# microsoft/GenerativeImage2Text

Hardware: AMD Instinct MI355X
Metric: captions/sec whole-node (GIT_BASE 224px bs=64/GPU greedy len=20) (higher is better)
Workload: dtype f16; 1 GPU; GIT_BASE 224px bs=64/GPU greedy max_len=20 frames=1; global_batch=64, parallelism=dp1, decode_steps_per_caption=19, seq_len_returned=20, hip_graph=True, contexts_in_flight=4, layernorm_folded=True, library=libgitmi_f16.so, encoder_chains=2, schedule=mixed

## Files before the change

### generativeimage2text_amd/csrc/abi_ops.hip

```cpp
#include "../../include/gitmi.h"
#include "abi_common.h"
#include "gitmi_common.h"
#include "launchers.h"

#include <hip/hip_runtime.h>

using namespace gitmi;

#ifdef GITMI_EXPERIMENT
#include "../../include/gitmi_experiment.h"
#define GITMI_EXP_EXPORT extern "C"
#else
#define GITMI_EXP_EXPORT [[maybe_unused]] static
#endif

static inline int round_up(int x, int m) { return (x + m - 1) / m * m; }

extern "C" int gitmi_operand_dtype(void);
static const char* dtype_name(int dtype) {
    return dtype == GITMI_DTYPE_F32 ? "fp32" : dtype == GITMI_DTYPE_BF16 ? "bf16" : dtype == GITMI_DTYPE_F16 ? "fp16" : "unknown";
}
static int check_dtype(const char* op, const char* arg, int dtype) {
    if (dtype == GITMI_DTYPE_F32 || dtype == gitmi_operand_dtype()) return 0;
    return fail("%s: %s is %s (%d), but this library's 16-bit operands are %s (libgitmi%s.so)", op, arg, dtype_name(dtype), dtype,
                dtype_name(gitmi_operand_dtype()), gitmi_operand_dtype() == GITMI_DTYPE_F16 ? "_f16" : "");
}

extern "C" int gitmi_op_gemm(const void* A, const void* W, const float* bias, const float* residual, void* C, int M,
                             int N, int K, int lda, int ldc, int in_dtype, int out_dtype, int act, void* stream) {
    GemmArgs g{};
    g.A = A; g.W = W; g.bias = bias; g.res = residual; g.C = C;
    g.M = M; g.N = N; g.K = K; g.lda = lda; g.ldc = ldc; g.ldr = ldc; g.act = act;
    RCK(check_dtype("op_gemm", "in_dtype", in_dtype));
    const bool in_f32 = in_dtype == GITMI_DTYPE_F32;
    if ((in_f32 && K % 16) || (!in_f32 && K % 64)) return fail("op_gemm: K must be a multiple of %d", in_f32 ? 16 : 64);
    if (out_dtype == GITMI_DTYPE_F16_STREAM) {
        if (in_f32) return fail("op_gemm: fp16 stream rows need 16-bit operands");
        g.out_f16 = 1;
    } else {
        RCK(check_dtype("op_gemm", "out_dtype", out_dtype));
    }
    HIPCK(launch_gemm(g, in_f32, out_dtype == GITMI_DTYPE_F32, (hipStream_t)stream));
    return 0;
}
extern "C" int gitmi_op_gemm_ln(const void* A, const void* W, const float* bias, const float* colsum, const float* ln_part,
                                float ln_eps, const void* residual, const float* res_part, const float* res_gamma,
                                const float* res_beta, float res_eps, void* C, float* part_out, int M, int N, int K, int act,
                                void* stream) {
    GemmArgs g{};
    g.A = A; g.W = W; g.bias = bias; g.C = C;
    g.M = M; g.N = N; g.K = K; g.lda = K; g.ldc = N; g.ldr = N; g.act = act;
    if (K % 64) return fail("op_gemm_ln: K must be a multiple of 64");
    if (ln_part) {
        if (!colsum || residual || part_out || res_part) return fail("op_gemm_ln: consumer form takes colsum and no residual / partial output");
        g.ln_part = (const float2*)ln_part; g.ln_nparts = (K + 255) / 256; g.ln_colsum = colsum; g.ln_inv_d = 1.0f / (float)K; g.ln_eps = ln_eps;
    } else {
        if (!part_out && !res_part) return fail("op_gemm_ln: neither a consumer (ln_part) nor a producer (part_out / res_part)");
        g.out_f16 = 1;
        g.res = (const float*)residual;
        g.part_out = (float2*)part_out;
        if (res_part) {
            g.res_part = (const float2*)res_part; g.res_nparts = (N + 255) / 256; g.res_gamma = res_gamma; g.res_beta = res_beta;
            g.res_inv_d = 1.0f / (float)N; g.res_eps = res_eps;
        }
    }
    if (!gemm_uses_p8(g, false, false))
        return fail("op_gemm_ln: the folded forms exist in gemm_p8_kernel only (more than 512 rows, N %% 256 == 0, K >= 128)");
    if (launch_gemm(g, false, false, (hipStream_t)stream) != hipSuccess)
        return fail("op_gemm_ln: launch refused (the folded forms are built into the fp16-operand library only)");
    return 0;
}
extern "C" int gitmi_op_layernorm(const float* x, const float* gamma, const float* beta, float eps, void* y_t,
                                  float* y_f32, int rows, int D, int out_dtype, void* stream) {
    if (y_t) RCK(check_dtype("op_layernorm", "out_dtype", out_dtype));
    HIPCK(launch_layernorm(x, D, gamma, beta, eps, nullptr, y_t, D, out_dtype == GITMI_DTYPE_F32, y_f32, D, rows, D, 0, 0,
                           0, (hipStream_t)stream));
    return 0;
}
extern "C" int gitmi_op_attention(const void* qkv, void* out, int B, int N, int H, int dtype, int impl, void* stream) {
    RCK(check_dtype("op_attention", "dtype", dtype));
    const size_t esz = dtype == GITMI_DTYPE_F32 ? 4 : 2;
    const int D = H * 64;
    AttnFullArgs a{};
    a.q = qkv;
    a.k = (const char*)qkv + (size_t)D * esz;
    a.v = (const char*)qkv + (size_t)2 * D * esz;
    a.out = out;
    a.ldq = a.ldk = a.ldv = 3 * D;
    a.ldo = D;
    a.N = N; a.H = H; a.scale = 0.125f;
    HIPCK(launch_attn_full(a, B, dtype == GITMI_DTYPE_F32, impl, (hipStream_t)stream));
    return 0;
}

#ifdef GITMI_EXPERIMENT
static int g_dgemm_dbg = 0;
GITMI_EXP_EXPORT int gitmi_debug_set_dgemm(int dbg) { g_dgemm_dbg = dbg; return 0; }
#else
static const int g_dgemm_dbg = 0;
#endif
extern "C" int gitmi_op_dgemm(const void* A, const void* W, const float* bias, const float* colsum, const float* stats,
                              int strips, float eps, void* C, int c_frag, int M, int N, int K, int act, int strips_per_wg,
                              void* stream) {
    if (c_frag && N % 32) return fail("op_dgemm: a fragment-major output needs N %% 32 == 0");
    const DLn ln{(const float2*)stats, strips, 1.0f / (float)K, eps, nullptr, nullptr};
    DGemmArgs g = dgemm_ln(A, W, bias, colsum, stats ? &ln : nullptr, C, c_frag, act, M, N, K);
    g.dbg = g_dgemm_dbg;
    g.strips_per_wg = strips_per_wg;
    if (K % 32) return fail("op_dgemm: K must be a multiple of 32");
    HIPCK(launch_dgemm(g, (hipStream_t)stream));
    return 0;
}
extern "C" int gitmi_op_dgemm_res(const void* A, const void* W, const float* bias, const float* res_x, const float* res_stats,
                                  int res_strips, const float* res_gamma, const float* res_beta, float res_eps,
                                  float* x_out, void* xb_out, float* stats_out, int M, int N, int K, void* stream) {
    const DLn res_ln{(const float2*)res_stats, res_strips, 1.0f / (float)N, res_eps, res_gamma, res_beta};
    DGemmArgs g = dgemm_to_stream(A, W, bias, res_x, res_stats ? &res_ln : nullptr, x_out, xb_out, (float2*)stats_out, M, N, K);
    g.dbg = g_dgemm_dbg;
    if (K % 32 || N % 16) return fail("op_dgemm_res: need K %% 32 == 0 and N %% 16 == 0");
    HIPCK(launch_dgemm(g, (hipStream_t)stream));
    return 0;
}
GITMI_EXP_EXPORT int gitmi_debug_dgemm_form(const void* A, int a_rows, const void* W, const float* bias, const float* colsum,
                                            const float* stats, int strips, float eps, void* C, int c_frag, int act,
                                            const float* res_x, const float* res_stats, int res_strips, const float* res_gamma,
                                            const float* res_beta, float res_eps, float* x_out, void* xb_out, float* stats_out,
                                            int M, int N, int K, int rows_per_wg, int strips_per_wg, int no_row_walk,
                                            void* stream) {
    if (!A || !W || !bias) return fail("debug_dgemm_form: null argument (A, W, bias)");
    if (M < 0 || N < 0 || K < 0) return fail("debug_dgemm_form: M=%d N=%d K=%d", M, N, K);
    if ((C != nullptr) == (x_out != nullptr)) return fail("debug_dgemm_form: exactly one of C and x_out selects the epilogue");
    if (K % 32) return fail("debug_dgemm_form: K must be a multiple of 32 (K=%d)", K);
    if (a_rows < round_up(M, 64)) return fail("debug_dgemm_form: a_rows=%d, but M=%d rows are loaded as %d", a_rows, M, round_up(M, 64));
    if (rows_per_wg < 0 || strips_per_wg < 0) return fail("debug_dgemm_form: rows_per_wg=%d strips_per_wg=%d", rows_per_wg, strips_per_wg);
    DGemmArgs g;
    if (C) {
        if (res_x || res_stats || xb_out || stats_out) return fail("debug_dgemm_form: residual arguments with the C epilogue");
        if (c_frag && N % 32) return fail("debug_dgemm_form: c_frag needs N %% 32 == 0 (N=%d)", N);
        if (stats) {
            if (!colsum) return fail("debug_dgemm_form: stats without colsum");
            if (strips < 1 || strips > 64) return fail("debug_dgemm_form: strips=%d outside [1, 64]", strips);
        }
        const DLn ln{(const float2*)stats, strips, 1.0f / (float)K, eps, nullptr, nullptr};
        g = dgemm_ln(A, W, bias, colsum, stats ? &ln : nullptr, C, c_frag, act, M, N, K);
    } else {
        if (stats || colsum || c_frag || act) return fail("debug_dgemm_form: consumer arguments with the x_out epilogue");
        if (N % 16) return fail("debug_dgemm_form: the x_out epilogue needs N %% 16 == 0 (N=%d)", N);
        if (!xb_out || !stats_out || !res_x) return fail("debug_dgemm_form: the x_out epilogue needs xb_out, stats_out and res_x");
        if (res_stats) {
            if (!res_gamma || !res_beta) return fail("debug_dgemm_form: res_stats without res_gamma / res_beta");
            if (res_strips < 1 || res_strips > 64) return fail("debug_dgemm_form: res_strips=%d outside [1, 64]", res_strips);
        }
        const DLn res_ln{(const float2*)res_stats, res_strips, 1.0f / (float)N, res_eps, res_gamma, res_beta};
        g = dgemm_to_stream(A, W, bias, res_x, res_stats ? &res_ln : nullptr, x_out, xb_out, (float2*)stats_out, M, N, K);
    }
    g.rows_per_wg = rows_per_wg; g.strips_per_wg = strips_per_wg; g.no_row_walk = no_row_walk;
    HIPCK(launch_dgemm(g, (hipStream_t)stream));
    return 0;
}
static VocabArgs vocab_op_args(const void* A, const void* W, const float* bias, const float* colsum, const float* stats, int strips,
                               float eps, int M, int V, int K, int cols_per_wg, float* part_val, int* part_idx, float* part_lse,
                               float* logits_out, int max_wgs) {
    VocabArgs v{};
    v.max_wgs = max_wgs;
    v.A = (const unsigned short*)A; v.lda = K; v.W = (const unsigned short*)W; v.bias = bias;
// ... 95 lines not shown
        HIPCK(hipMemcpy(node.data(), child_node, node.size() * sizeof(int), hipMemcpyDeviceToHost));
        for (int i = 0; i < n_edges; ++i)
            if (node[i] < 0 || node[i] >= n_nodes) return fail("debug_trie_select: edge %d leads to node %d of %d", i, node[i], n_nodes);
    }
    HIPCK(hipMemcpy(cur.data(), cursor, cur.size() * sizeof(int), hipMemcpyDeviceToHost));
    for (int b = 0; b < B; ++b)
        if (cur[b] < -1 || cur[b] >= n_nodes) return fail("debug_trie_select: cursor %d of sentence %d outside [-1, %d)", cur[b], b, n_nodes);
    const TrieArgs tr{child_off, child_tok, child_node, cursor};
    HIPCK(launch_trie_select(logits, ldl, V, ids, ld_ids, cur_len, plen, eos, tr, B, part_val, part_idx, (float2*)part_lse, s));
    return 0;
}
GITMI_EXP_EXPORT int gitmi_debug_sample_rows(const float* logits, int R, int V, float temperature, int top_k, float top_p, int ndraw,
                                             uint64_t seed, int step, float* draw_logprob, int* draw_token, float* filtered_out,
                                             int ldl, const int* ids, int ld_ids, int cur_len, float rep_penalty, int stride,
                                             void* stream) {
    if (!logits || !draw_logprob || !draw_token) return fail("debug_sample_rows: null argument");
    if (R < 1 || V < 1 || ldl < V) return fail("debug_sample_rows: R=%d V=%d ldl=%d", R, V, ldl);
    RCK(check_history("debug_sample_rows", ids, ld_ids, cur_len));
    float2* lse = nullptr;
    HIPCK(hipMalloc((void**)&lse, (size_t)R * sizeof(float2)));
    hipError_t err = launch_sample_rows(logits, ldl, V, R, temperature, top_k, top_p, ndraw, seed, step, draw_logprob, draw_token, lse,
                                        filtered_out, ids, ld_ids, cur_len, rep_penalty, stride, (hipStream_t)stream);
    if (err == hipSuccess) err = hipStreamSynchronize((hipStream_t)stream);
    hipFree(lse);
    HIPCK(err);
    return 0;
}

GITMI_EXP_EXPORT int gitmi_debug_set_gemm_impl(int impl) {
    if (!set_gemm_impl(impl)) return fail("debug_set_gemm_impl: unknown selector %d (low byte: -1, 0 or 9)", impl);
    return 0;
}

GITMI_EXP_EXPORT int gitmi_debug_gemm_form(const void* A, int lda, const void* W, const float* bias, const void* res, int ldr, void* C,
                                           int ldc, int M, int N, int K, int act, int in_dtype, int out_dtype, int shared,
                                           const float* ln_part, const float* colsum, float ln_eps, float* part_out,
                                           const float* res_part, const float* res_gamma, const float* res_beta, float res_eps,
                                           void* stream) {
    if (!A || !W || !C) return fail("debug_gemm_form: null argument (A, W, C)");
    if (M < 0 || N < 1 || K < 1) return fail("debug_gemm_form: M=%d N=%d K=%d", M, N, K);
    if (lda < K) return fail("debug_gemm_form: lda=%d < K=%d", lda, K);
    if (ldc < N) return fail("debug_gemm_form: ldc=%d < N=%d", ldc, N);
    if (res && ldr < N) return fail("debug_gemm_form: ldr=%d < N=%d", ldr, N);
    if (act < GITMI_ACT_NONE || act > GITMI_ACT_GELU_ERF) return fail("debug_gemm_form: act=%d", act);
    RCK(check_dtype("debug_gemm_form", "in_dtype", in_dtype));
    const bool in_f32 = in_dtype == GITMI_DTYPE_F32;
    if ((in_f32 && K % 16) || (!in_f32 && K % 64)) return fail("debug_gemm_form: K must be a multiple of %d (K=%d)", in_f32 ? 16 : 64, K);
    GemmArgs g{};
    g.A = A; g.W = W; g.bias = bias; g.res = (const float*)res; g.C = C;
    g.M = M; g.N = N; g.K = K; g.lda = lda; g.ldc = ldc; g.ldr = res ? ldr : 0; g.act = act;
    g.shared = shared ? 1 : 0;
    if (out_dtype == GITMI_DTYPE_F16_STREAM) {
        if (in_f32) return fail("debug_gemm_form: fp16 stream rows need 16-bit operands");
        g.out_f16 = 1;
    } else {
        RCK(check_dtype("debug_gemm_form", "out_dtype", out_dtype));
    }
    const bool out_f32 = out_dtype == GITMI_DTYPE_F32;
    const bool consumer = ln_part != nullptr, producer = part_out != nullptr || res_part != nullptr;
    if (colsum && !consumer) return fail("debug_gemm_form: colsum without ln_part");
    if ((res_gamma || res_beta) && !res_part) return fail("debug_gemm_form: res_gamma / res_beta without res_part");
    if (consumer || producer) {
#ifndef GITMI_OPS_F16
        return fail("debug_gemm_form: the folded-LayerNorm forms are built into the fp16-operand library only");
#endif
        if (consumer && producer) return fail("debug_gemm_form: consumer (ln_part) and producer (part_out / res_part) arguments in one launch");
        if (consumer) {
            if (!colsum) return fail("debug_gemm_form: ln_part without colsum");
            if (res || in_f32 || out_f32 || g.out_f16) return fail("debug_gemm_form: the consumer writes operand-type rows and takes no residual");
            if (K > 1024) return fail("debug_gemm_form: row partials cover K <= 1024 (K=%d)", K);
            g.ln_part = (const float2*)ln_part; g.ln_nparts = (K + 255) / 256; g.ln_colsum = colsum; g.ln_inv_d = 1.0f / (float)K; g.ln_eps = ln_eps;
        } else {
            if (!g.out_f16 || act != GITMI_ACT_NONE) return fail("debug_gemm_form: the producer writes fp16 stream rows and has no activation");
            if (N > 1024) return fail("debug_gemm_form: row partials cover N <= 1024 (N=%d)", N);
            g.part_out = (float2*)part_out;
            if (res_part) {
                if (!res || !res_gamma || !res_beta) return fail("debug_gemm_form: res_part without res / res_gamma / res_beta");
                g.res_part = (const float2*)res_part; g.res_nparts = (N + 255) / 256; g.res_gamma = res_gamma; g.res_beta = res_beta;
                g.res_inv_d = 1.0f / (float)N; g.res_eps = res_eps;
            }
        }
        if (!gemm_uses_p8(g, false, false))
            return fail("debug_gemm_form: the folded forms exist in gemm_p8_kernel only (more than 512 rows, N %% 256 == 0, K >= 128, 16-byte aligned rows)");
    }
    HIPCK(launch_gemm(g, in_f32, out_f32, (hipStream_t)stream));
    return 0;
}

extern "C" int gitmi_op_attn_decode(const void* qkv, const void* img_k, const void* img_v, void* txt_k, void* txt_v,
                                    const int* kv_src, void* out, int B, int H, int N_img, int T_max, int pos, int beams,
                                    int dtype, int dbg, void* stream) {
    RCK(check_dtype("op_attn_decode", "dtype", dtype));
    AttnDecodeArgs a{};
    a.qkv = qkv; a.img_k = img_k; a.img_v = img_v; a.txt_k = txt_k; a.txt_v = txt_v; a.out = out;
    a.kv_src = kv_src; a.ld_src = T_max; a.d = H * 64; a.N_img = N_img; a.T_max = T_max; a.pos = pos; a.beams = beams;
    a.scale = 0.125f; a.dbg = dbg & 0xffff; a.waves_per_pair = (dbg >> 16) & 3; a.stream_wgs = dbg >> 18;
    if (dtype == GITMI_DTYPE_F32) {
        HIPCK(launch_attn_decode(a, B, H, (hipStream_t)stream));
        return 0;
    }
    a.N_pad = round_up(N_img, 32);
    HIPCK(launch_attn_decode_mfma(a, B, H, (hipStream_t)stream));
    return 0;
}
extern "C" int gitmi_op_kv_repack(const void* qkv_rows, void* kf, void* vt, int B, int N, int H, void* stream) {
    HIPCK(launch_kv_repack_frag(qkv_rows, kf, vt, B, N, round_up(N, 32), H, H * 64, (hipStream_t)stream));
    return 0;
}

GITMI_EXP_EXPORT int gitmi_debug_attention_ragged(const void* qkv, void* out, const int* ntok, int B, int N, int H, int dtype, int impl,
                                                  void* stream) {
    if (!ntok) return fail("debug_attention_ragged: ntok is required");
    const size_t esz = dtype == GITMI_DTYPE_F32 ? 4 : 2;
    const int D = H * 64;
    AttnFullArgs a{};
    a.q = qkv;
    a.k = (const char*)qkv + (size_t)D * esz;
    a.v = (const char*)qkv + (size_t)2 * D * esz;
    a.out = out;
    a.ldq = a.ldk = a.ldv = 3 * D;
    a.ldo = D;
    a.N = N; a.H = H; a.scale = 0.125f; a.ntok = ntok;
    HIPCK(launch_attn_full(a, B, dtype == GITMI_DTYPE_F32, impl, (hipStream_t)stream));
    return 0;
}
GITMI_EXP_EXPORT int gitmi_debug_attn_decode_form(const void* qkv, const void* img_k, const void* img_v, void* txt_k, void* txt_v,
                                                  const int* kv_src, void* out, const int* ntok, const int* img_of, int n_images,
                                                  int B, int H, int N_img, int T_max, int pos, int beams, int dtype, int out_frag,
                                                  int pairs_per_wg, int waves_per_pair, int stream_wgs, void* stream) {
    RCK(check_dtype("debug_attn_decode_form", "dtype", dtype));
    if (!qkv || !img_k || !img_v || !txt_k || !txt_v || !kv_src || !out) return fail("debug_attn_decode_form: null argument");
    if (beams < 1 || beams > 8) return fail("debug_attn_decode_form: beams=%d outside [1, 8]", beams);
    if (n_images < 1) return fail("debug_attn_decode_form: n_images=%d", n_images);
    if (B < 1 || H < 1 || N_img < 1 || pos < 0 || pos >= T_max)
        return fail("debug_attn_decode_form: B=%d H=%d N_img=%d pos=%d T_max=%d", B, H, N_img, pos, T_max);
    if (out_frag && dtype == GITMI_DTYPE_F32) return fail("debug_attn_decode_form: out_frag needs 16-bit rows");
    if (ntok && stream_wgs > 0) return fail("debug_attn_decode_form: the streaming kernel does not serve ragged batches (ntok)");
    AttnDecodeArgs a{};
    a.qkv = qkv; a.img_k = img_k; a.img_v = img_v; a.txt_k = txt_k; a.txt_v = txt_v; a.out = out;
    a.kv_src = kv_src; a.ld_src = T_max; a.d = H * 64; a.N_img = N_img; a.T_max = T_max; a.pos = pos; a.beams = beams;
    a.scale = 0.125f; a.ntok = ntok; a.img_of = img_of; a.out_frag = out_frag;
    a.pairs_per_wg = pairs_per_wg; a.waves_per_pair = waves_per_pair; a.stream_wgs = stream_wgs;
    if (dtype == GITMI_DTYPE_F32) {
        HIPCK(launch_attn_decode(a, B, H, (hipStream_t)stream));
        return 0;
    }
    a.N_pad = round_up(N_img, 32);
    HIPCK(launch_attn_decode_mfma(a, B, H, (hipStream_t)stream));
    return 0;
}
GITMI_EXP_EXPORT int gitmi_debug_attn_decode_qkv(const void* x, int x_rows, const void* w, const float* bias, const float* colsum,
                                                 const float* stats, int strips, float eps, const void* img_k, const void* img_v,
                                                 void* txt_k, void* txt_v, const int* kv_src, void* out, const int* ntok,
                                                 const int* img_of, int n_images, int B, int H, int N_img, int T_max, int pos,
                                                 int beams, int dtype, int out_frag, int pairs_per_wg, int waves_per_pair,
                                                 int stream_wgs, void* stream) {
    RCK(check_dtype("debug_attn_decode_qkv", "dtype", dtype));
    if (dtype == GITMI_DTYPE_F32) return fail("debug_attn_decode_qkv: 16-bit operands only (the f32 mode keeps its QKV launch)");
    if (!x || !w || !bias || !img_k || !img_v || !txt_k || !txt_v || !kv_src || !out) return fail("debug_attn_decode_qkv: null argument");
    if (n_images < 1) return fail("debug_attn_decode_qkv: n_images=%d", n_images);
    if (B < 1 || H < 1 || N_img < 1 || pos < 0 || pos >= T_max)
        return fail("debug_attn_decode_qkv: B=%d H=%d N_img=%d pos=%d T_max=%d", B, H, N_img, pos, T_max);
    if (beams != 1) return fail("debug_attn_decode_qkv: beams=%d (beam batches keep the QKV launch)", beams);
    if (ntok) return fail("debug_attn_decode_qkv: ntok (ragged batches keep the QKV launch)");
    if (waves_per_pair == 2) return fail("debug_attn_decode_qkv: waves_per_pair=2 (two-wave pairs keep the QKV launch)");
    if (stream_wgs != 0) return fail("debug_attn_decode_qkv: stream_wgs=%d (the streaming form keeps the QKV launch)", stream_wgs);
// ... 247 lines not shown
```

### generativeimage2text_amd/csrc/engine.hip

```cpp
#include "../../include/gitmi.h"
#include "engine_state.h"

#include <algorithm>
#include <cmath>
#include <cstdarg>
#include <cstdio>
#include <cstring>

using namespace gitmi;

#ifdef GITMI_EXPERIMENT
#include "../../include/gitmi_experiment.h"
#define GITMI_EXP_EXPORT extern "C"
#else
#define GITMI_EXP_EXPORT [[maybe_unused]] static
#endif

static thread_local char g_err[1024] = "";
int gitmi::fail(const char* fmt, ...) {
    va_list ap;
    va_start(ap, fmt);
    vsnprintf(g_err, sizeof(g_err), fmt, ap);
    va_end(ap);
    return 1;
}

static hipEvent_t get_event(gitmi_engine* e) {
    if (e->event_next == e->event_pool.size()) {
        hipEvent_t ev;
        hipEventCreate(&ev);
        e->event_pool.push_back(ev);
    }
    return e->event_pool[e->event_next++];
}
struct SpanGuard {
    gitmi_engine* e; hipStream_t s; size_t idx; bool on;
    SpanGuard(gitmi_engine* e_, hipStream_t s_, int tag, double flops) : e(e_), s(s_), idx(0), on(e_->profiling) {
        if (!on) return;
        TimedSpan sp{get_event(e), get_event(e), tag, flops};
        hipEventRecord(sp.a, s);
        idx = e->spans.size();
        e->spans.push_back(sp);
    }
    ~SpanGuard() { if (on) hipEventRecord(e->spans[idx].b, s); }
};

static bool gemm_tall_tiles(const gitmi_engine* e, int N) {
    if (!e->pol.shared_device) return false;
    return e->pol.gemm_tall == 1 || (e->pol.gemm_tall == 2 && N >= 2048) || (e->pol.gemm_tall == 3 && N < 2048);
}

static double gemm_flops(int M, int N, int K) { return 2.0 * (double)M * (double)N * (double)K; }
static GemmArgs gemm_args(const void* A, int lda, const void* W, const float* bias, const void* res, int ldr, void* C, int ldc,
                          int M, int N, int K, int act) {
    GemmArgs g{};
    g.A = A; g.W = W; g.bias = bias; g.res = (const float*)res; g.C = C;
    g.M = M; g.N = N; g.K = K; g.lda = lda; g.ldc = ldc; g.ldr = ldr; g.act = act;
    return g;
}
static int gemm_run(gitmi_engine* e, hipStream_t s, GemmArgs g, bool in_f32, bool out_f32, int tag) {
    g.shared = gemm_tall_tiles(e, g.N) ? 1 : 0;
    SpanGuard sp(e, s, tag, gemm_flops(g.M, g.N, g.K));
    HIPCK(launch_gemm(g, in_f32, out_f32, s));
    return 0;
}
static int gemm(gitmi_engine* e, hipStream_t s, const void* A, int lda, const void* W, const float* bias,
                const float* res, int ldr, void* C, int ldc, bool out_f32, int M, int N, int K, int act, int tag) {
    return gemm_run(e, s, gemm_args(A, lda, W, bias, res, ldr, C, ldc, M, N, K, act), e->pol.f32, out_f32, tag);
}
static bool on_p8(const void* A, int lda, const void* W, const void* C, int ldc, int M, int N, int K, bool stream_out) {
    GemmArgs g = gemm_args(A, lda, W, nullptr, nullptr, 0, const_cast<void*>(C), ldc, M, N, K, 0);
    g.out_f16 = stream_out ? 1 : 0;
    return gemm_uses_p8(g, false, false);
}
struct Stream {
    void* x = nullptr; int M = 0, D = 0, tag = 0;
    bool fold = false;
    void* t = nullptr;
    float* xn = nullptr;
    float2* parts[2] = {nullptr, nullptr};
    const float2* part = nullptr; const float* gamma = nullptr; const float* beta = nullptr; float eps = 0.f;
};
static float2* stream_part_out(const Stream& st) { return st.part == st.parts[0] ? st.parts[1] : st.parts[0]; }
static void stream_written(Stream& st, const float2* part, const float* gamma, const float* beta, float eps) {
    st.part = part; st.gamma = gamma; st.beta = beta; st.eps = eps;
}
static int ln_gemm(gitmi_engine* e, hipStream_t s, const Stream& st, const Folded& f, const void* W, const float* bias, void* C,
                   int ldc, int col0, int N, int act) {
    const int D = st.D;
    const size_t woff = (size_t)col0 * D * e->pol.esz;
    C = (char*)C + (size_t)col0 * e->pol.esz;
    if (st.fold) {
        GemmArgs g = gemm_args(st.x, D, (const char*)f.w + woff, f.bias + col0, nullptr, 0, C, ldc, st.M, N, D, act);
        g.ln_part = st.part; g.ln_nparts = D / 256; g.ln_colsum = f.colsum + col0; g.ln_inv_d = 1.0f / (float)D; g.ln_eps = st.eps;
        return gemm_run(e, s, g, false, false, st.tag);
    }
    if (e->pol.stream_f16)
        HIPCK(launch_layernorm_s16(st.x, D, st.gamma, st.beta, st.eps, nullptr, st.t, D, false, st.xn, st.xn ? D : 0, st.M, D, 0, 0, 0, s));
    else
        HIPCK(launch_layernorm((const float*)st.x, D, st.gamma, st.beta, st.eps, nullptr, st.t, D, e->pol.f32, st.xn, st.xn ? D : 0, st.M,
                               D, 0, 0, 0, s));
    return gemm(e, s, st.t, D, (const char*)W + woff, bias + col0, nullptr, 0, C, ldc, e->pol.f32, st.M, N, D, act, st.tag);
}
static int gemm_to_stream(gitmi_engine* e, hipStream_t s, Stream& st, const void* A, int lda, const void* W, const float* bias, int K,
                          bool residual, const float* gamma, const float* beta, float eps) {
    const int D = st.D;
    float2* part = gamma ? stream_part_out(st) : nullptr;
    const void* res = !residual ? nullptr : st.xn && !st.fold ? st.xn : st.x;
    GemmArgs g = gemm_args(A, lda, W, bias, res, residual ? D : 0, st.x, D, st.M, D, K, 0);
    g.out_f16 = e->pol.stream_f16 ? 1 : 0;
    if (st.fold) {
        g.part_out = part;
        if (residual && st.xn) {
            g.res_part = st.part; g.res_nparts = D / 256; g.res_gamma = st.gamma; g.res_beta = st.beta;
            g.res_inv_d = 1.0f / (float)D; g.res_eps = st.eps;
        }
    }
    RCK(gemm_run(e, s, g, e->pol.f32, !e->pol.stream_f16, st.tag));
    stream_written(st, part, gamma, beta, eps);
    return 0;
}
static int attn_full_packed(gitmi_engine* e, const void* qkv, void* out, int width, int heads, int N, int batch, const int* ntok,
                            hipStream_t s) {
    AttnFullArgs a{};
    a.q = qkv;
    a.k = (const char*)qkv + (size_t)width * e->pol.esz;
    a.v = (const char*)qkv + (size_t)2 * width * e->pol.esz;
    a.out = out;
    a.ldq = a.ldk = a.ldv = 3 * width;
    a.ldo = width;
    a.N = N; a.H = heads; a.scale = 0.125f;
    a.ntok = ntok;
    HIPCK(launch_attn_full(a, batch, e->pol.f32, e->pol.attn_impl, s));
    return 0;
}
static int dec_layer_tail(gitmi_engine* e, hipStream_t s, const DecLayerW& L, const void* ctx, float* hf, void* ht, float* y, void* u,
                          int M) {
    const int d = e->cfg.dec_hidden, ffn = e->cfg.dec_ffn;
    RCK(gemm(e, s, ctx, d, L.wo, L.bo, hf, d, y, d, true, M, d, d, 0, TAG_GEMM_OTHER));
    HIPCK(launch_layernorm(y, d, L.lnag, L.lnab, 1e-12f, nullptr, ht, d, e->pol.f32, hf, d, M, d, 0, 0, 0, s));
    RCK(gemm(e, s, ht, d, L.w1, L.b1, nullptr, 0, u, ffn, e->pol.f32, M, ffn, d, 2, TAG_GEMM_OTHER));
    RCK(gemm(e, s, u, ffn, L.w2, L.b2, hf, d, y, d, true, M, d, ffn, 0, TAG_GEMM_OTHER));
    HIPCK(launch_layernorm(y, d, L.lnog, L.lnob, 1e-12f, nullptr, ht, d, e->pol.f32, hf, d, M, d, 0, 0, 0, s));
    return 0;
}

extern "C" int gitmi_abi_version(void) { return GITMI_ABI_VERSION; }
extern "C" int gitmi_operand_dtype(void) {
#ifdef GITMI_OPS_F16
    return GITMI_DTYPE_F16;
#else
    return GITMI_DTYPE_BF16;
#endif
}
extern "C" const char* gitmi_last_error(void) { return g_err; }

extern "C" int gitmi_create(const gitmi_config* cfg, int device, gitmi_engine** out) {
    if (!cfg || !out) return fail("gitmi_create: null argument");
    int ndev = 0;
    if (hipGetDeviceCount(&ndev) != hipSuccess || ndev <= 0)
        return fail("gitmi_create: no HIP device available (this engine has no CPU fallback)");
    if (device < 0 || device >= ndev) return fail("gitmi_create: device %d out of range (%d devices)", device, ndev);
    HIPCK(hipSetDevice(device));
    hipDeviceProp_t prop;
    HIPCK(hipGetDeviceProperties(&prop, device));
    if (strncmp(prop.gcnArchName, "gfx950", 6) != 0)
        return fail("gitmi_create: device %d is %s; this library is built for gfx950 (MI355X) only", device,
                    prop.gcnArchName);
    const gitmi_config& c = *cfg;
    if (c.vit_width % c.vit_heads || c.vit_width / c.vit_heads != 64) return fail("ViT head_dim must be 64");
    if (c.dec_hidden % c.dec_heads || c.dec_hidden / c.dec_heads != 64) return fail("decoder head_dim must be 64");
    if (c.image_size % c.patch) return fail("image_size must be a multiple of patch");
    if (c.max_image_pixels < 0 || c.max_image_tokens < 0) return fail("negative image capacity");
    if (c.vit_width > 1024 || c.dec_hidden > 1024) return fail("hidden sizes above 1024 are not supported");
    if (c.vit_width % 64 || c.dec_hidden % 64 || c.dec_ffn % 64) return fail("hidden sizes must be multiples of 64");
    if (c.max_batch < 1 || c.max_beams < 1 || c.max_beams > 8 || c.max_frames < 1 || c.max_text_len < 2)
        return fail("bad capacity (max_batch>=1, 1<=max_beams<=8, max_frames>=1, max_text_len>=2)");
    if (c.max_text_len > c.max_pos) return fail("max_text_len exceeds max_pos");
    if (c.precision != GITMI_PREC_BF16 && c.precision != GITMI_PREC_F32) return fail("bad precision");

    gitmi_engine* e = new gitmi_engine();
    e->cfg = c;
    e->device = device;
    e->pol.f32 = c.precision == GITMI_PREC_F32;
    e->pol.esz = e->pol.f32 ? 4 : 2;
    e->pol.attn_impl = e->pol.f32 ? 0 : 1;
    init_geometry(e);
    e->pol.stream_f16 = !e->pol.f32;
#ifdef GITMI_OPS_F16
    e->pol.ln_fold = !e->pol.f32 && c.vit_width % 256 == 0 && c.dec_hidden % 256 == 0;
#endif
#ifdef GITMI_EXPERIMENT
    if (const char* env = getenv("GITMI_ATTN_IMPL")) e->pol.attn_impl = e->pol.f32 ? 0 : atoi(env);
    if (const char* env = getenv("GITMI_GRAPH")) e->pol.use_graph = atoi(env) != 0;
    if (const char* env = getenv("GITMI_ATTN_DBG")) e->pol.attn_dbg = atoi(env);
    if (const char* env = getenv("GITMI_ATTN_PW")) e->pol.attn_pw = atoi(env);
    if (const char* env = getenv("GITMI_ATTN_NH")) e->pol.attn_nh = atoi(env);
    if (const char* env = getenv("GITMI_ATTN_STREAM")) e->pol.attn_stream = atoi(env);
    if (const char* env = getenv("GITMI_DECODE_SKIP")) e->pol.decode_skip = atoi(env);
    if (const char* env = getenv("GITMI_GEMM_TALL")) e->pol.gemm_tall = atoi(env);
    if (const char* env = getenv("GITMI_DGEMM_ROWS")) e->pol.dgemm_rows = atoi(env);
    if (const char* env = getenv("GITMI_DGEMM_STRIPS")) e->pol.dgemm_strips = atoi(env);
    if (const char* env = getenv("GITMI_DGEMM_NO_ROW_WALK")) e->pol.dgemm_no_row_walk = atoi(env);
    if (const char* env = getenv("GITMI_DGEMM_DBG")) e->pol.dgemm_dbg = atoi(env);
    if (const char* env = getenv("GITMI_VOCAB_WGS")) e->pol.vocab_wgs = atoi(env);
    if (const char* env = getenv("GITMI_SKINNY")) e->pol.skinny = atoi(env) != 0;
    if (const char* env = getenv("GITMI_STREAM_F16")) e->pol.stream_f16 = !e->pol.f32 && atoi(env) != 0;
    if (const char* env = getenv("GITMI_GEMM_IMPL")) set_gemm_impl(atoi(env));
#endif
    e->pol.ln_fold = e->pol.ln_fold && e->pol.stream_f16;
    e->pol.ln_fold_ready = e->pol.ln_fold;
    *out = e;
    return 0;
}

int CapturedGraph::capture(hipStream_t s, const std::function<int()>& fn) {
    reset();
    HIPCK(hipStreamBeginCapture(s, hipStreamCaptureModeThreadLocal));
    const int rc = fn();
    const hipError_t ce = hipStreamEndCapture(s, &graph);
    if (rc != 0 || ce != hipSuccess) reset();
    RCK(rc);
    HIPCK(ce);
    HIPCK(hipGraphInstantiate(&exec, graph, nullptr, nullptr, 0));
    return 0;
}
static void destroy_graph(gitmi_engine* e) {
    for (CapturedGraph* g : {&e->graph_full, &e->graph_decode, &e->graph_follow}) g->reset();
    e->full_slot.valid = e->follow_slot.valid = false;
}
static void drop_resident(gitmi_engine* e) { e->have_feats = e->have_prefill = false; }
static void set_resident(gitmi_engine* e, int B, int F_eff, int stride = 0) {
    e->cur_B = B; e->cur_F = F_eff; e->cur_Nimg = stride > 0 ? stride : F_eff * e->N;
    e->have_feats = true; e->have_prefill = false;
    e->keyed = e->ragged; e->has_context = false;
    e->res_desc.clear();
}
static void set_context(gitmi_engine* e) { e->keyed = e->has_context = true; }
static const int* key_counts(const gitmi_engine* e) { return e->keyed ? e->rg_ntok : nullptr; }
static void set_prefilled(gitmi_engine* e) { e->have_prefill = true; }
static int settle_residency(gitmi_engine* e, const Request& rq, int rc) {
    if (rc != 0 && rq.frames) drop_resident(e);
    return rc;
}

extern "C" void gitmi_destroy(gitmi_engine* e) {
    if (!e) return;
    hipSetDevice(e->device);
    hipDeviceSynchronize();
    if (e->enc_after) {
        auto& w = e->enc_after->enc_watchers;
        w.erase(std::remove(w.begin(), w.end(), e), w.end());
    }
    for (gitmi_engine* w : e->enc_watchers) w->enc_after = nullptr;
    destroy_graph(e);
    if (e->own_stream) hipStreamDestroy(e->own_stream);
    if (e->fence_in) hipEventDestroy(e->fence_in);
    if (e->fence_out) hipEventDestroy(e->fence_out);
    for (auto ev : e->gev)
        if (ev) hipEventDestroy(ev);
    if (e->enc_done) hipEventDestroy(e->enc_done);
    for (auto ev : e->event_pool) hipEventDestroy(ev);
    for (void* p : e->allocs) hipFree(p);
    for (void* p : e->sc_allocs) hipFree(p);
    hipFree(e->at_out); hipFree(e->at_stats); hipFree(e->ctx_tab); hipFree(e->mem_tab); hipFree(e->feat_tab); hipFree(e->ban_words);
    if (e->ban_stage) hipHostFree(e->ban_stage);
    if (e->ban_staged) hipEventDestroy(e->ban_staged);
    if (e->trie_off) hipFree(e->trie_off);
    if (e->trie_tok) hipFree(e->trie_tok);
    if (e->trie_child) hipFree(e->trie_child);
    delete e;
}

extern "C" int gitmi_set_image_shape(gitmi_engine* e, int H, int W, void* stream) {
    if (!e) return fail("null engine");
    if (!e->finalized) return fail("weights not finalized");
    const gitmi_config& c = e->cfg;
    if (H == 0 && W == 0) {
        if (!e->ragged) {
            e->ragged = true;
            e->H = e->W = e->gh = e->gw = 0;
            e->N = e->Nmax;
            drop_resident(e);
        }
        return 0;
    }
    if (H < c.patch || W < c.patch) return fail("image %dx%d is smaller than one %d-pixel patch", H, W, c.patch);
    const int gh = H / c.patch, gw = W / c.patch;
    if ((size_t)H * W > e->max_pixels)
        return fail("image %dx%d exceeds the max_image_pixels capacity (%zu)", H, W, e->max_pixels);
    if (gh * gw + 1 > e->Nmax)
        return fail("a %dx%d token grid exceeds the max_image_tokens capacity (%d)", gh, gw, e->Nmax);
    if (H == e->H && W == e->W && !e->ragged) return 0;
    e->ragged = false;
    HIPCK(hipSetDevice(e->device));
    if (gh == e->g_nat && gw == e->g_nat) {
        e->pos_cur = e->w.pos;
    } else {
        HIPCK(launch_pos_bicubic(e->w.pos, e->pos_var, e->g_nat, gh, gw, c.vit_width, (hipStream_t)stream));
        e->pos_cur = e->pos_var;
    }
    e->H = H; e->W = W; e->gh = gh; e->gw = gw; e->N = gh * gw + 1;
    drop_resident(e);
    return 0;
}

static Stream vit_stream(gitmi_engine* e, int M) {
    const int D = e->cfg.vit_width;
    const VitLayerW& L = e->w.vit[0];
    Stream st;
    st.x = e->v_x; st.M = M; st.D = D; st.tag = TAG_GEMM_VIT; st.t = e->v_h;
    st.fold = e->pol.ln_fold && on_p8(e->v_x, D, L.qkv_f.w, e->v_qkv, 3 * D, M, 3 * D, D, false) &&
              on_p8(e->v_x, D, L.ffn1_f.w, e->v_u, 4 * D, M, 4 * D, D, false) && on_p8(e->v_ctx, D, L.wo, e->v_x, D, M, D, D, true) &&
              on_p8(e->v_u, 4 * D, L.w2, e->v_x, D, M, D, 4 * D, true);
    if (st.fold) st.parts[0] = st.parts[1] = e->v_part;
    return st;
}
static Stream prefill_stream(gitmi_engine* e, int M) {
    const int d = e->cfg.dec_hidden, ffn = e->cfg.dec_ffn, D = e->cfg.vit_width;
    const DecLayerW& L = e->w.dec[0];
    Stream st;
    st.x = e->p_y; st.M = M; st.D = d; st.tag = TAG_GEMM_OTHER; st.t = e->p_ht; st.xn = e->p_hf;
    st.fold = e->pol.ln_fold && on_p8(e->feats, D, e->w.vp_w, e->p_y, d, M, d, D, true) &&
              on_p8(e->p_y, d, L.qkv_pf.w, e->img_kv[0], 3 * d, M, 3 * d, d, false) &&
              on_p8(e->p_y, d, L.qkv_pf.w, e->img_kv[0], 3 * d, M, 2 * d, d, false) &&
              (e->cfg.dec_layers < 2 || (on_p8(e->p_y, d, L.ffn1_pf.w, e->p_u, ffn, M, ffn, d, false) &&
                                         on_p8(e->p_ctx, d, L.wo, e->p_y, d, M, d, d, true) && on_p8(e->p_u, ffn, L.w2, e->p_y, d, M, d, ffn, true)));
    if (st.fold) { st.parts[0] = e->p_part[0]; st.parts[1] = e->p_part[1]; }
    return st;
}

static int encode_frames_impl(gitmi_engine* e, const float* const* frames, int F, int B, float* feats_out,
                              hipStream_t s, int stride = 0) {
    const gitmi_config& c = e->cfg;
    const int D = c.vit_width, N = e->N;
    const int F_eff = c.num_frames > 0 ? std::min(F, c.num_frames) : F;
    const int Nimg = stride > 0 ? stride : F_eff * N;
    drop_resident(e);
    SpanGuard phase(e, s, TAG_VIT, 0);
    const int BI = F_eff * B;
    const int M = BI * N;
    const int g2 = N - 1;
    const size_t slot = (size_t)3 * e->max_pixels;
    if (e->ragged)
        HIPCK(launch_im2col_ragged(e->frame_stage[0], slot, e->rg_meta, e->patches, e->pol.f32, B, N, c.patch, e->Kp, e->Kp_pad, s));
    else
    for (int fr = 0; fr < F_eff; ++fr)
        HIPCK(launch_im2col(frames[fr], (char*)e->patches + (size_t)fr * B * g2 * e->Kp_pad * e->pol.esz, e->pol.f32, B,
                            e->H, e->W, c.patch, e->Kp, e->Kp_pad, s));
    RCK(gemm(e, s, e->patches, e->Kp_pad, e->w.conv_w, nullptr, nullptr, 0, e->patch_out, D, true, BI * g2, D, e->Kp_pad, 0,
             TAG_GEMM_VIT));
    Stream x = vit_stream(e, M);
    float2* part = stream_part_out(x);
    if (e->ragged)
        HIPCK(launch_vit_assemble_ragged(e->patch_out, e->w.cls, e->w.pos, e->g_nat, e->rg_meta, e->w.lnpre_g, e->w.lnpre_b, 1e-5f, e->v_x,
                                         e->pol.stream_f16, BI, N, c.patch, D, part, s));
    else
    HIPCK(launch_vit_assemble_ln(e->patch_out, e->w.cls, e->pos_cur, e->w.lnpre_g, e->w.lnpre_b, 1e-5f, e->v_x, e->pol.stream_f16, BI, N, D,
                                 part, D / 256, s));
    stream_written(x, part, e->w.vit[0].ln1g, e->w.vit[0].ln1b, 1e-5f);
    for (int l = 0; l < c.vit_layers; ++l) {
        const VitLayerW& L = e->w.vit[l];
        const VitLayerW* Ln = l + 1 < c.vit_layers ? &e->w.vit[l + 1] : nullptr;
        RCK(ln_gemm(e, s, x, L.qkv_f, L.wqkv, L.bqkv, e->v_qkv, 3 * D, 0, 3 * D, 0));
        RCK(attn_full_packed(e, e->v_qkv, e->v_ctx, D, c.vit_heads, N, BI, e->ragged ? e->rg_ntok : nullptr, s));
        RCK(gemm_to_stream(e, s, x, e->v_ctx, D, L.wo, L.bo, D, true, L.ln2g, L.ln2b, 1e-5f));
        RCK(ln_gemm(e, s, x, L.ffn1_f, L.w1, L.b1, e->v_u, 4 * D, 0, 4 * D, 1));
        RCK(gemm_to_stream(e, s, x, e->v_u, 4 * D, L.w2, L.b2, 4 * D, true, Ln ? Ln->ln1g : nullptr, Ln ? Ln->ln1b : nullptr, 1e-5f));
    }
    for (int fr = 0; fr < F_eff; ++fr) {
        const float* te = (c.num_frames > 0 && e->pol.use_temb) ? e->w.temb[fr] : nullptr;
        if (e->pol.stream_f16) {
            const char* xs = (const char*)e->v_x + (size_t)fr * B * N * D * 2;
            HIPCK(launch_layernorm_s16(xs, D, e->w.lnpost_g, e->w.lnpost_b, 1e-5f, te, e->feats, D, false, nullptr, 0, B * N, D, N,
                                       Nimg, fr * N, s));
            if (feats_out)
                HIPCK(launch_layernorm_s16(xs, D, e->w.lnpost_g, e->w.lnpost_b, 1e-5f, te, feats_out, D, true, nullptr, 0, B * N, D,
                                           N, Nimg, fr * N, s));
        } else {
            HIPCK(launch_layernorm(e->v_x + (size_t)fr * B * N * D, D, e->w.lnpost_g, e->w.lnpost_b, 1e-5f, te, e->feats, D, e->pol.f32,
                                   feats_out, D, B * N, D, N, Nimg, fr * N, s));
        }
    }
    if (e->ragged) {
        HIPCK(launch_zero_pad_rows(e->feats, e->pol.f32, D, e->rg_ntok, B, N, s));
        if (feats_out) HIPCK(launch_zero_pad_rows(feats_out, true, D, e->rg_ntok, B, N, s));
    }

    set_resident(e, B, F_eff, stride);
    return 0;
}

static int kv_repack(gitmi_engine* e, int l, int B, int Nimg, hipStream_t s) {
    const gitmi_config& c = e->cfg;
    void* kh = e->img_kh[l];
    void* vh = e->img_vh[l];
    if (e->pol.f32) HIPCK(launch_kv_repack(e->img_kv[l], kh, vh, B, Nimg, c.dec_heads, c.dec_hidden, s));
    else HIPCK(launch_kv_repack_frag(e->img_kv[l], kh, vh, B, Nimg, round_up(Nimg, 32), c.dec_heads, c.dec_hidden, s));
    return 0;
}

static int prefill_impl(gitmi_engine* e, hipStream_t s) {
    const gitmi_config& c = e->cfg;
    const int d = c.dec_hidden, ffn = c.dec_ffn, D = c.vit_width;
    const int B = e->cur_B, Nimg = e->cur_Nimg, M = B * Nimg;
    e->have_prefill = false;
    SpanGuard phase(e, s, TAG_PREFILL, 0);
    Stream y = prefill_stream(e, M);
    RCK(gemm_to_stream(e, s, y, e->feats, D, e->w.vp_w, e->w.vp_b, D, false, e->w.vp_lng, e->w.vp_lnb, 1e-5f));
    for (int l = 0; l < c.dec_layers; ++l) {
        const DecLayerW& L = e->w.dec[l];
        const bool last = l + 1 == c.dec_layers;
        const int col0 = last ? d : 0;
        RCK(ln_gemm(e, s, y, L.qkv_pf, L.wqkv, L.bqkv, e->img_kv[l], 3 * d, col0, 3 * d - col0, 0));
        RCK(kv_repack(e, l, B, Nimg, s));
        if (last) break;
        RCK(attn_full_packed(e, e->img_kv[l], e->p_ctx, d, c.dec_heads, Nimg, B, key_counts(e), s));
        RCK(gemm_to_stream(e, s, y, e->p_ctx, d, L.wo, L.bo, d, true, L.lnag, L.lnab, 1e-12f));
        RCK(ln_gemm(e, s, y, L.ffn1_pf, L.w1, L.b1, e->p_u, ffn, 0, ffn, 2));
        RCK(gemm_to_stream(e, s, y, e->p_u, ffn, L.w2, L.b2, ffn, true, L.lnog, L.lnob, 1e-12f));
    }
    set_prefilled(e);
    return 0;
}

#ifdef GITMI_EXPERIMENT
#define GITMI_SKIPPED(e, bit) (((e)->pol.decode_skip & (bit)) != 0)
#else
#define GITMI_SKIPPED(e, bit) false
#endif
static int dgemm(gitmi_engine* e, hipStream_t s, const DGemmArgs& g_in) {
    DGemmArgs g = g_in;
    g.dbg = e->pol.dgemm_dbg;
    g.no_row_walk = e->pol.dgemm_no_row_walk >= 0 ? e->pol.dgemm_no_row_walk : e->pol.shared_device ? 0 : 1;
    g.strips_per_wg = e->pol.dgemm_strips >= 0 ? e->pol.dgemm_strips : e->pol.shared_device ? 2 : 1;
    g.rows_per_wg = e->pol.dgemm_rows > 0 ? e->pol.dgemm_rows : g.M > 64 ? 64 : e->pol.shared_device ? 32 : 16;
    SpanGuard sp(e, s, TAG_GEMM_OTHER, gemm_flops(g.M, g.N, g.K));
    HIPCK(launch_dgemm(g, s));
    return 0;
}

static DGemmArgs dgemm_ln(const void* A, const Folded& f, const DLn* ln, void* C, int c_frag, int act, int M, int N, int K) {
    return dgemm_ln(A, f.w, f.bias, f.colsum, ln, C, c_frag, act, M, N, K);
}

static int decode_layers_impl(gitmi_engine* e, const int* kv_src, int ld_ids, int pos, int R, int beams, hipStream_t s) {
    const gitmi_config& c = e->cfg;
    const int d = c.dec_hidden, ffn = c.dec_ffn;
    const int B = R / beams;
    const bool chain = e->pol.skinny && !e->pol.f32;
    for (int l = 0; l < c.dec_layers; ++l) {
        const DecLayerW& L = e->w.dec[l];
        const DecLayerW* Lp = l > 0 ? &e->w.dec[l - 1] : nullptr;
        const DLn ln_prev{e->stats_o, d / 16, 1.0f / (float)d, 1e-12f, Lp ? Lp->lnog : nullptr, Lp ? Lp->lnob : nullptr};
        const DLn ln_a{e->stats_a, d / 16, 1.0f / (float)d, 1e-12f, L.lnag, L.lnab};
        const DLn* ln_o = Lp ? &ln_prev : nullptr;
        AttnDecodeArgs a{};
        a.qkv = e->d_qkv; a.img_k = e->img_kh[l]; a.img_v = e->img_vh[l]; a.txt_k = e->txt_k[l]; a.txt_v = e->txt_v[l]; a.out = e->d_ctx;
        a.kv_src = kv_src; a.ld_src = ld_ids; a.d = d; a.N_img = e->cur_Nimg; a.T_max = c.max_text_len;
        a.img_of = e->img_identity ? nullptr : e->img_of_dev;
        a.pos = pos; a.beams = beams; a.scale = 0.125f;
        a.out_frag = chain ? 1 : 0;
        a.N_pad = round_up(e->cur_Nimg, 32);
        a.dbg = e->pol.attn_dbg;
        a.waves_per_pair = e->pol.attn_nh;
        a.pairs_per_wg = e->pol.attn_pw > 0 ? e->pol.attn_pw : e->pol.shared_device ? 8 : 4;
        const bool stream_ok = !e->pol.shared_device && a.N_pad <= 8 * 32 && B * c.dec_heads >= 384 && e->pol.attn_nh != 2;
        a.stream_wgs = e->pol.attn_stream >= 0 ? e->pol.attn_stream : stream_ok ? 192 : 0;
        if (e->keyed) { a.ntok = e->rg_ntok; a.stream_wgs = 0; }
        bool qkv_inside = false;
        if (chain) {
            const DGemmArgs g = dgemm_ln(l == 0 ? e->d_ht : e->xo_b, L.qkv_f, ln_o, e->d_qkv, 0, 0, R, 3 * d, d);
            attn_decode_set_qkv(a, g);
            qkv_inside = !GITMI_SKIPPED(e, ~0) && !e->pol.dgemm_dbg && attn_decode_qkv_form(a, B, c.dec_heads) && attn_decode_pairs_per_wg(a, B, c.dec_heads) == 8;
            if (!qkv_inside && !GITMI_SKIPPED(e, 2) && !GITMI_SKIPPED(e, 16)) RCK(dgemm(e, s, g));
        } else {
            RCK(gemm(e, s, e->d_ht, d, L.wqkv, L.bqkv, nullptr, 0, e->d_qkv, 3 * d, e->pol.f32, R, 3 * d, d, 0, TAG_GEMM_OTHER));
        }
        if (e->pol.f32) HIPCK(launch_attn_decode(a, B, c.dec_heads, s));
        else if (qkv_inside) HIPCK(launch_attn_decode_qkv(a, B, c.dec_heads, s));
        else if (!GITMI_SKIPPED(e, 1)) HIPCK(launch_attn_decode_mfma(a, B, c.dec_heads, s));
        if (chain) {
            if (!GITMI_SKIPPED(e, 4))
                RCK(dgemm(e, s, dgemm_to_stream(e->d_ctx, L.wo_p, L.bo, l == 0 ? e->d_hf : e->xo_f, ln_o, e->xa_f, e->xa_b, e->stats_a, R, d, d)));
            if (!GITMI_SKIPPED(e, 2)) RCK(dgemm(e, s, dgemm_ln(e->xa_b, L.ffn1_f, &ln_a, e->d_u, 1, 2, R, ffn, d)));
            if (!GITMI_SKIPPED(e, 4))
                RCK(dgemm(e, s, dgemm_to_stream(e->d_u, L.w2_p, L.b2, e->xa_f, &ln_a, e->xo_f, e->xo_b, e->stats_o, R, d, ffn)));
        } else {
            RCK(dec_layer_tail(e, s, L, e->d_ctx, e->d_hf, e->d_ht, e->d_y, e->d_u, R));
        }
    }
    return 0;
}

static int sample_candidates(gitmi_engine* e, const float* logits, int ldl, int R, int step, hipStream_t s, StepCands* cands,
                             const BanArgs* ban);
static int trie_candidates(gitmi_engine* e, const float* logits, int ldl, int cur_len, hipStream_t s, StepCands* cands);
static float rep_penalty_of(const gitmi_engine* e) {
    const double rp = e->sample.repetition_penalty;
    return (e->ss.kind == GITMI_SEARCH_GENERATOR && rp > 0 && rp != 1.0) ? (float)rp : 0.f;
}
// ... 1321 lines not shown
```

### generativeimage2text_amd/csrc/engine_state.h

```cpp
#pragma once
#include "../../include/gitmi.h"
#include "abi_common.h"
#include "launchers.h"

#include <hip/hip_runtime.h>

#include <functional>
#include <map>
#include <string>
#include <tuple>
#include <vector>

static inline int round_up(int x, int m) { return (x + m - 1) / m * m; }
static inline int keep_best(const gitmi_search& sp) { return sp.num_keep_best > 1 ? sp.num_keep_best : 1; }

struct HostTensor {
    std::vector<float> data;
    std::vector<int64_t> shape;
    float amax = 0.f;
    size_t numel() const { size_t n = 1; for (auto s : shape) n *= (size_t)s; return n; }
};

struct Folded { void* w = nullptr; float* bias = nullptr; float* colsum = nullptr; };

struct VitLayerW {
    void *wqkv = nullptr, *wo = nullptr, *w1 = nullptr, *w2 = nullptr;
    float *bqkv = nullptr, *bo = nullptr, *b1 = nullptr, *b2 = nullptr;
    float *ln1g = nullptr, *ln1b = nullptr, *ln2g = nullptr, *ln2b = nullptr;
    Folded qkv_f;
    Folded ffn1_f;
};
struct DecLayerW {
    void *wqkv = nullptr, *wo = nullptr, *w1 = nullptr, *w2 = nullptr;
    float *bqkv = nullptr, *bo = nullptr, *b1 = nullptr, *b2 = nullptr;
    float *lnag = nullptr, *lnab = nullptr, *lnog = nullptr, *lnob = nullptr;
    Folded qkv_f;
    Folded ffn1_f;
    void *wo_p = nullptr, *w2_p = nullptr;
    Folded qkv_pf, ffn1_pf;
};

struct TimedSpan { hipEvent_t a, b; int tag; double flops; };
enum { TAG_VIT = 0, TAG_PREFILL = 1, TAG_DECODE = 2, TAG_GEMM_VIT = 10, TAG_GEMM_OTHER = 11, TAG_STEP = 20 };

struct GraphKey {
    int B, Q, F, P, kind, k, pn, T, H, W, prefixed, ident, temb, resident, Nimg, keyed; double lp;
    int smp, top_k, nh; double top_p, temp, rp; unsigned long long seed;
    int constrained;
    auto fields() const {
        return std::tie(B, Q, F, P, kind, k, pn, T, H, W, prefixed, ident, temb, resident, Nimg, keyed, lp, smp, top_k, nh, top_p, temp,
                        rp, seed, constrained);
    }
    bool operator==(const GraphKey& o) const { return fields() == o.fields(); }
};
struct GraphSlot { GraphKey key{}; bool valid = false; };

struct CapturedGraph {
    hipGraph_t graph = nullptr;
    hipGraphExec_t exec = nullptr;
    void reset() {
        if (exec) hipGraphExecDestroy(exec);
        if (graph) hipGraphDestroy(graph);
        exec = nullptr, graph = nullptr;
    }
    int capture(hipStream_t s, const std::function<int()>& fn);
    hipError_t launch(hipStream_t s) const { return hipGraphLaunch(exec, s); }
};

struct Request {
    const float* const* frames;
    int F, B, Q, minP, maxP;
    bool prefixed;
    const gitmi_search* sp;
    long long* tokens; float* logprob; int32_t* info;
    int32_t* sent;
};

struct ModelWeights {
    void* conv_w = nullptr;
    float *cls = nullptr, *pos = nullptr, *lnpre_g = nullptr, *lnpre_b = nullptr, *lnpost_g = nullptr, *lnpost_b = nullptr;
    std::vector<VitLayerW> vit;
    std::vector<float*> temb;
    void* vp_w = nullptr;
    float *vp_b = nullptr, *vp_lng = nullptr, *vp_lnb = nullptr;
    float *words_f = nullptr, *positions_f = nullptr, *emb_lng = nullptr, *emb_lnb = nullptr;
    std::vector<DecLayerW> dec;
    void* out_w = nullptr;
    float* out_b = nullptr;
    Folded out_f;
    double dec_weight_bytes = 0;
};

struct Policy {
    bool f32 = false;
    size_t esz = 2;
    int attn_impl = 1;
    bool stream_f16 = false;
    bool ln_fold = false;
    bool ln_fold_ready = false;
    bool skinny = true;
    bool use_graph = true;
    bool use_temb = true;
    bool shared_device = false;
    int attn_dbg = 0, dgemm_dbg = 0;
    int attn_pw = 0;
    int attn_nh = 0;
    int attn_stream = -1;
    int dgemm_no_row_walk = -1;
    int dgemm_strips = -1;
    int vocab_wgs = -1;
    int gemm_tall = 1;
    int dgemm_rows = 0;
    int decode_skip = 0;
};

struct gitmi_engine {
    gitmi_config cfg{};
    ModelWeights w;
    Policy pol;
    int device = 0;
    bool finalized = false;
    gitmi_engine* parent = nullptr;

    std::map<std::string, HostTensor> host_w;
    std::vector<void*> allocs;

    int N = 0, gh = 0, gw = 0, H = 0, W = 0, Kp = 0, Kp_pad = 0;
    int N_nat = 0, g_nat = 0, Nmax = 0;
    size_t max_pixels = 0;
    float* pos_var = nullptr;
    const float* pos_cur = nullptr;
    bool ragged = false;
    int4* rg_meta = nullptr;
    int* rg_ntok = nullptr;
    bool keyed = false;
    bool has_context = false;
    int* ctx_tab = nullptr;
    size_t ctx_tab_ints = 0;
    gitmi::MemoryEntry* mem_tab = nullptr;
    size_t mem_tab_n = 0;
    std::vector<int4> res_desc;
    gitmi::FeaturePiece* feat_tab = nullptr;
    unsigned int* ban_words = nullptr;
    int* ban_stage = nullptr;
    hipEvent_t ban_staged = nullptr;
    int ban_armed = 0;
    bool ban_live = false;

    void *patches = nullptr, *v_h = nullptr, *v_qkv = nullptr, *v_ctx = nullptr, *v_u = nullptr;
    float *patch_out = nullptr, *v_x = nullptr;
    void* feats = nullptr;
    float *p_y = nullptr, *p_hf = nullptr;
    void *p_ht = nullptr, *p_ctx = nullptr, *p_u = nullptr;
    std::vector<void*> img_kv;
    std::vector<void*> img_kh, img_vh;
    float *d_y = nullptr, *d_hf = nullptr, *logits = nullptr;
    void *d_ht = nullptr, *d_qkv = nullptr, *d_ctx = nullptr, *d_u = nullptr;
    std::vector<void*> txt_k, txt_v;
    int ldl = 0;
    float *xa_f = nullptr, *xo_f = nullptr;
    void *xa_b = nullptr, *xo_b = nullptr;
    float2 *stats_a = nullptr, *stats_o = nullptr;
    float* part_val = nullptr; int* part_idx = nullptr; float2* part_lse = nullptr;
    int vocab_cols = 128, vocab_nparts = 1;
    gitmi::SearchState ss{};
    int ss_cur = 0, ss_len = 0;
    long long* start_dev = nullptr;
    int *plen_dev = nullptr, *img_of_dev = nullptr;
    bool img_identity = true;
    int *trie_off = nullptr, *trie_tok = nullptr, *trie_child = nullptr, *trie_cursor = nullptr;
    bool trie_search = false;
    gitmi_search sample{};
    std::vector<int> plen_host, img_of_host;

    int cur_B = 0, cur_F = 0, cur_Nimg = 0;
    bool have_feats = false, have_prefill = false;

    int profile_mode = 0;
    bool profiling = false;
    float2 *v_part = nullptr, *p_part[2] = {nullptr, nullptr};
    hipEvent_t gev[3] = {nullptr, nullptr, nullptr};
    gitmi_engine* enc_after = nullptr;
    std::vector<gitmi_engine*> enc_watchers;
    hipEvent_t enc_done = nullptr;
    double split_encode_ms = 0, split_decode_ms = 0;
    int split_calls = 0, split_steps = 0;
    std::vector<TimedSpan> spans;
    std::vector<hipEvent_t> event_pool;
    size_t event_next = 0;
    double last_decode_step_bytes = 0;

    CapturedGraph graph_full, graph_decode, graph_follow;
    GraphSlot full_slot, follow_slot;
    bool graph_is_split = false;
    std::vector<float*> frame_stage;
    long long* out_tokens = nullptr;
    float* out_lp = nullptr;
    int* out_info = nullptr;
    int* out_sent = nullptr;
    hipStream_t own_stream = nullptr;
    hipEvent_t fence_in = nullptr, fence_out = nullptr;

    size_t sc_rows = 0;
    std::vector<void*> sc_allocs;
    float *sc_hf = nullptr, *sc_y = nullptr, *sc_zt = nullptr;
    void *sc_ht = nullptr, *sc_qkv = nullptr, *sc_ctx = nullptr, *sc_u = nullptr;
    float4* sc_part = nullptr;
    int *sc_tgt = nullptr, *sc_lens = nullptr, *sc_img = nullptr, *sc_bad = nullptr, *sc_info = nullptr;
    float2* sc_out = nullptr;
    size_t tr_out_n = 0;
    int* tr_nodes = nullptr;
    float2* tr_out = nullptr;
    size_t at_floats = 0, at_stat_rows = 0;
    float* at_out = nullptr;
    float2* at_stats = nullptr;
};

namespace gitmi {
void init_geometry(gitmi_engine* e);
}
```

### generativeimage2text_amd/csrc/engine_weights.hip

```cpp
#include "engine_state.h"

#include <algorithm>
#include <cmath>
#include <cstring>

using namespace gitmi;

static int dev_alloc(gitmi_engine* e, void** p, size_t bytes) {
    if (bytes == 0) bytes = 16;
    HIPCK(hipMalloc(p, bytes));
    e->allocs.push_back(*p);
    return 0;
}
template <typename T> static int dev_alloc_t(gitmi_engine* e, T** p, size_t count) {
    return dev_alloc(e, reinterpret_cast<void**>(p), count * sizeof(T));
}

static float half_to_float(uint16_t h) {
    const uint32_t sign = (uint32_t)(h & 0x8000) << 16;
    uint32_t exp = (h >> 10) & 0x1f, man = h & 0x3ff, out;
    if (exp == 0) {
        if (man == 0) out = sign;
        else {
            exp = 127 - 15 + 1;
// ... 41 lines not shown
}

static int get_w(gitmi_engine* e, const std::string& key, std::initializer_list<int64_t> shape, const HostTensor** out) {
    auto it = e->host_w.find(key);
    if (it == e->host_w.end()) return fail("missing weight '%s'", key.c_str());
    size_t want = 1;
    for (auto s : shape) want *= (size_t)s;
    if (it->second.numel() != want) return fail("weight '%s' has %zu elements, expected %zu", key.c_str(), it->second.numel(), want);
    *out = &it->second;
    return 0;
}
static int up_f32(gitmi_engine* e, const std::string& key, std::initializer_list<int64_t> shape, float** dst) {
    const HostTensor* t;
    RCK(get_w(e, key, shape, &t));
    RCK(dev_alloc_t(e, dst, t->numel()));
    HIPCK(hipMemcpy(*dst, t->data.data(), t->numel() * 4, hipMemcpyHostToDevice));
    return 0;
}
static int operand_range_check(gitmi_engine* e, const char* what, float amax) {
#ifdef GITMI_OPS_F16
    if (!e->pol.f32 && amax > 65504.f)
        return fail("'%s': max |w| = %g is outside the fp16 operand range (65504): load this checkpoint with precision "
                    "\"bf16\" or \"f32\"", what, (double)amax);
#endif
    (void)e; (void)what; (void)amax;
    return 0;
}
static int up_mat(gitmi_engine* e, const std::string& key, int64_t rows, int K, int Kpad, void** dst) {
    const HostTensor* t;
    RCK(get_w(e, key, {rows, (int64_t)K}, &t));
    RCK(operand_range_check(e, key.c_str(), t->amax));
    RCK(dev_alloc(e, dst, (size_t)rows * Kpad * e->pol.esz));
    float* tmp = nullptr;
    HIPCK(hipMalloc((void**)&tmp, t->numel() * 4));
    hipError_t err = hipMemcpy(tmp, t->data.data(), t->numel() * 4, hipMemcpyHostToDevice);
    if (err == hipSuccess) err = launch_convert_pad(tmp, *dst, e->pol.f32, (size_t)rows, K, Kpad, 0);
    if (err == hipSuccess) err = hipDeviceSynchronize();
    hipFree(tmp);
    HIPCK(err);
    return 0;
}

void gitmi::init_geometry(gitmi_engine* e) {
    const gitmi_config& c = e->cfg;
    e->g_nat = e->gh = e->gw = c.image_size / c.patch;
    e->N_nat = e->N = e->g_nat * e->g_nat + 1;
    e->H = e->W = c.image_size;
    e->Nmax = std::max(e->N_nat, c.max_image_tokens);
    e->max_pixels = std::max((size_t)c.image_size * c.image_size, (size_t)c.max_image_pixels);
    e->Kp = 3 * c.patch * c.patch;
    e->Kp_pad = round_up(e->Kp, 64);
    e->pos_cur = e->w.pos;
}

static int alloc_workspaces(gitmi_engine* e) {
    const gitmi_config& c = e->cfg;
    const size_t esz = e->pol.esz;
    const int D = c.vit_width, d = c.dec_hidden;
    const size_t Mv = (size_t)c.max_batch * c.max_frames * e->Nmax;
    const size_t Mp = (size_t)c.max_batch * c.max_frames * e->Nmax;
    const size_t R = (size_t)round_up(c.max_batch * c.max_beams, 64);
    const int T = c.max_text_len;
    RCK(dev_alloc(e, &e->patches, (size_t)c.max_batch * c.max_frames * (e->Nmax - 1) * e->Kp_pad * esz));
    RCK(dev_alloc_t(e, &e->patch_out, (size_t)c.max_batch * c.max_frames * (e->Nmax - 1) * D));
    RCK(dev_alloc_t(e, &e->pos_var, (size_t)e->Nmax * D));
    RCK(dev_alloc_t(e, &e->v_x, Mv * D));
    RCK(dev_alloc(e, &e->v_h, Mv * D * esz));
    RCK(dev_alloc(e, &e->v_qkv, Mv * 3 * D * esz));
    RCK(dev_alloc(e, &e->v_ctx, Mv * D * esz));
    RCK(dev_alloc(e, &e->v_u, Mv * 4 * D * esz));
    RCK(dev_alloc(e, &e->feats, Mp * D * esz));
    if (e->pol.ln_fold_ready) {
        RCK(dev_alloc_t(e, &e->v_part, Mv * 4));
        RCK(dev_alloc_t(e, &e->p_part[0], Mp * 4));
        RCK(dev_alloc_t(e, &e->p_part[1], Mp * 4));
        HIPCK(hipMemset(e->v_part, 0, Mv * 4 * sizeof(float2)));
        HIPCK(hipMemset(e->p_part[0], 0, Mp * 4 * sizeof(float2)));
        HIPCK(hipMemset(e->p_part[1], 0, Mp * 4 * sizeof(float2)));
    }
    RCK(dev_alloc_t(e, &e->p_y, Mp * d));
    RCK(dev_alloc_t(e, &e->p_hf, Mp * d));
    RCK(dev_alloc(e, &e->p_ht, Mp * d * esz));
    RCK(dev_alloc(e, &e->p_ctx, Mp * d * esz));
    RCK(dev_alloc(e, &e->p_u, Mp * c.dec_ffn * esz));
    e->img_kv.resize(c.dec_layers);
    e->img_kh.resize(c.dec_layers);
    e->img_vh.resize(c.dec_layers);
    e->txt_k.resize(c.dec_layers);
    e->txt_v.resize(c.dec_layers);
    for (int l = 0; l < c.dec_layers; ++l) {
        RCK(dev_alloc(e, &e->img_kv[l], Mp * 3 * d * esz));
        const size_t Mkv = (size_t)c.max_batch * round_up(c.max_frames * e->Nmax, 32);
        RCK(dev_alloc(e, &e->img_kh[l], Mkv * d * esz));
        RCK(dev_alloc(e, &e->img_vh[l], Mkv * d * esz));
        RCK(dev_alloc(e, &e->txt_k[l], R * T * d * esz));
        RCK(dev_alloc(e, &e->txt_v[l], R * T * d * esz));
    }
    RCK(dev_alloc_t(e, &e->d_y, R * d));
    RCK(dev_alloc_t(e, &e->d_hf, R * d));
    RCK(dev_alloc(e, &e->d_ht, R * d * esz));
    RCK(dev_alloc(e, &e->d_qkv, R * 3 * d * esz));
    RCK(dev_alloc(e, &e->d_ctx, R * d * esz));
    RCK(dev_alloc(e, &e->d_u, R * c.dec_ffn * esz));
    RCK(dev_alloc_t(e, &e->xa_f, R * d));
    RCK(dev_alloc_t(e, &e->xo_f, R * d));
    RCK(dev_alloc(e, &e->xa_b, R * d * 2));
    RCK(dev_alloc(e, &e->xo_b, R * d * 2));
    RCK(dev_alloc_t(e, &e->stats_a, R * (size_t)(d / 16)));
    RCK(dev_alloc_t(e, &e->stats_o, R * (size_t)(d / 16)));
    e->ldl = round_up(c.vocab, 8);
    RCK(dev_alloc_t(e, &e->logits, R * e->ldl));
    e->vocab_cols = 128;
    e->vocab_nparts = (e->pol.skinny && !e->pol.f32) ? vocab_parts(c.vocab, e->vocab_cols) : 1;
    RCK(dev_alloc_t(e, &e->part_val, R * (size_t)e->vocab_nparts * 16));
    RCK(dev_alloc_t(e, &e->part_idx, R * (size_t)e->vocab_nparts * 16));
    RCK(dev_alloc_t(e, &e->part_lse, R * (size_t)e->vocab_nparts));
    SearchState& s = e->ss;
    for (int i = 0; i < 2; ++i) {
        RCK(dev_alloc_t(e, &s.ids[i], R * T));
        RCK(dev_alloc_t(e, &s.kv_src[i], R * T));
        RCK(dev_alloc_t(e, &s.score[i], R));
    }
    RCK(dev_alloc_t(e, &s.done, (size_t)c.max_batch));
    RCK(dev_alloc_t(e, &s.hyp_n, (size_t)c.max_batch));
    RCK(dev_alloc_t(e, &s.hyp_cnt, (size_t)c.max_batch));
    RCK(dev_alloc_t(e, &s.hyp_worst, (size_t)c.max_batch));
    RCK(dev_alloc_t(e, &s.hyp_score, (size_t)c.max_batch * SS_NHMAX));
    RCK(dev_alloc_t(e, &s.hyp_len, (size_t)c.max_batch * SS_NHMAX));
    RCK(dev_alloc_t(e, &s.hyp_seq, (size_t)c.max_batch * SS_NHMAX));
    RCK(dev_alloc_t(e, &s.hyp_tok, (size_t)c.max_batch * SS_NHMAX * T));
    RCK(dev_alloc_t(e, &s.stop, (size_t)c.max_batch));
    RCK(dev_alloc_t(e, &s.early, (size_t)c.max_batch));
    RCK(dev_alloc_t(e, &s.info, 4));
    RCK(dev_alloc_t(e, &s.len_norm, (size_t)T + 1));
    RCK(dev_alloc_t(e, &e->start_dev, (size_t)c.max_batch * T));
    RCK(dev_alloc_t(e, &e->plen_dev, (size_t)c.max_batch));
    RCK(dev_alloc_t(e, &e->img_of_dev, (size_t)c.max_batch));
    RCK(dev_alloc_t(e, &e->trie_cursor, (size_t)c.max_batch));
    RCK(dev_alloc_t(e, &e->out_tokens, (size_t)c.max_batch * SS_NHMAX * T));
    RCK(dev_alloc_t(e, &e->out_lp, (size_t)c.max_batch * SS_NHMAX));
    RCK(dev_alloc_t(e, &e->out_info, 4));
    RCK(dev_alloc_t(e, &e->out_sent, (size_t)c.max_batch * 2));
    HIPCK(hipStreamCreateWithFlags(&e->own_stream, hipStreamNonBlocking));
    HIPCK(hipEventCreateWithFlags(&e->fence_in, hipEventDisableTiming));
    HIPCK(hipEventCreateWithFlags(&e->fence_out, hipEventDisableTiming));
    e->frame_stage.resize(c.max_frames);
    for (int f = 0; f < c.max_frames; ++f)
        RCK(dev_alloc_t(e, &e->frame_stage[f], (size_t)c.max_batch * 3 * e->max_pixels));
    RCK(dev_alloc_t(e, &e->rg_meta, (size_t)c.max_batch));
    RCK(dev_alloc_t(e, &e->rg_ntok, (size_t)c.max_batch));
    return 0;
}

#ifdef GITMI_OPS_F16
static inline float bf16_round(float f) { return (float)(_Float16)f; }
#else
static inline float bf16_round(float f) {
    uint32_t u;
    memcpy(&u, &f, 4);
    if ((u & 0x7f800000u) == 0x7f800000u) return f;
    u += 0x7fffu + ((u >> 16) & 1u);
    u &= 0xffff0000u;
    memcpy(&f, &u, 4);
    return f;
}
#endif
// ... 216 lines not shown
```

### generativeimage2text_amd/csrc/kernels_attn.hip

```cpp
#include "gitmi_common.h"
#include "launchers.h"
#include <type_traits>

namespace gitmi {

constexpr int HD = 64;

template <typename T>
__global__ __launch_bounds__(256) void attn_full_valu_kernel(AttnFullArgs a) {
    __shared__ float Ks[64][HD + 1];
    __shared__ float Vs[64][HD + 1];
    __shared__ float qs[16][HD];
    __shared__ float ps[16][64];

    const int tid = threadIdx.x, lane = tid & 63, wave = tid >> 6;
    const int h = blockIdx.y, b = blockIdx.z;
    const int q0 = blockIdx.x * 16;
    const T* Q = reinterpret_cast<const T*>(a.q);
    const T* K = reinterpret_cast<const T*>(a.k);
    const T* V = reinterpret_cast<const T*>(a.v);
    T* O = reinterpret_cast<T*>(a.out);
    const size_t base_row = (size_t)b * a.N;
    const int n = a.ntok ? a.ntok[b] : a.N;
    if (q0 >= n) {
// ... 131 lines not shown
#pragma unroll
            for (int st_ = 0; st_ < 4; ++st_)
#pragma unroll
                for (int r = 0; r < 4; ++r) {
                    const int key = kt + st_ * 16 + lg * 4 + r;
                    const float sv = key < n ? s_acc[st_][r] * a.scale : -INFINITY;
                    s_acc[st_][r] = sv;
                    tmax = fmaxf(tmax, sv);
                }
            tmax = fmaxf(tmax, __shfl_xor(tmax, 16, 64));
            tmax = fmaxf(tmax, __shfl_xor(tmax, 32, 64));
            const float m_new = fmaxf(m_run[t], tmax);
            const float alpha = fast_exp(m_run[t] - m_new);
            float psum = 0.f;
#pragma unroll
            for (int st_ = 0; st_ < 4; ++st_)
#pragma unroll
                for (int r = 0; r < 4; ++r) {
                    const float p = fast_exp(s_acc[st_][r] - m_new);
                    s_acc[st_][r] = p;
                    psum += p;
                }
            psum += __shfl_xor(psum, 16, 64);
            psum += __shfl_xor(psum, 32, 64);
            l_run[t] = l_run[t] * alpha + psum;
            m_run[t] = m_new;
#pragma unroll
            for (int dt = 0; dt < 4; ++dt)
#pragma unroll
                for (int r = 0; r < 4; ++r) o_acc[t][dt][r] *= alpha;

#pragma unroll
            for (int hf = 0; hf < 2; ++hf) {
                bf16x8_t pf;
                {
                    union { bf16x8_t v; uint32_t u[4]; } pk;
                    pk.u[0] = pack2bf(s_acc[2 * hf][0], s_acc[2 * hf][1]);
                    pk.u[1] = pack2bf(s_acc[2 * hf][2], s_acc[2 * hf][3]);
                    pk.u[2] = pack2bf(s_acc[2 * hf + 1][0], s_acc[2 * hf + 1][1]);
                    pk.u[3] = pack2bf(s_acc[2 * hf + 1][2], s_acc[2 * hf + 1][3]);
                    pf = pk.v;
                }
#pragma unroll
                for (int dt = 0; dt < 4; ++dt) {
                    union { bf16x8_t v; uint2 h2[2]; } vf;
                    const bf16_t* vp = Vt + (dt * 16 + l15) * FA_LDV + hf * 32 + lg * 4;
                    vf.h2[0] = *reinterpret_cast<const uint2*>(vp);
                    vf.h2[1] = *reinterpret_cast<const uint2*>(vp + 16);
                    o_acc[t][dt] = mfma16(vf.v, pf, o_acc[t][dt]);
                }
            }
        }
    }

#pragma unroll
    for (int t = 0; t < QT; ++t) {
        const int qr = qbase + (t * 4 + wave) * 16 + l15;
        if (qr < a.N) {
            const float inv = qr < n ? 1.0f / l_run[t] : 0.f;
            bf16_t* op = O + (base_row + qr) * a.ldo + h * HD;
#pragma unroll
            for (int dt = 0; dt < 4; ++dt) {
                uint2 tt;
                tt.x = pack2bf(o_acc[t][dt][0] * inv, o_acc[t][dt][1] * inv);
                tt.y = pack2bf(o_acc[t][dt][2] * inv, o_acc[t][dt][3] * inv);
                *reinterpret_cast<uint2*>(op + dt * 16 + lg * 4) = tt;
            }
        }
    }
}

template <int NSUB, bool RAGGED = false>
__global__ __launch_bounds__(256, 2) void attn_full_mfma_short_kernel(AttnFullArgs a) {
    constexpr int NK = NSUB * 16;
    constexpr int NB = (NSUB + 1) / 2;
    constexpr int LDV = NB * 32 + 8;
    static_assert((LDV / 8) % 2 == 1, "V^T row stride must be an odd multiple of 16 bytes");
    __shared__ __attribute__((aligned(16))) bf16_t Ks[NK * FA_LDK];
    __shared__ __attribute__((aligned(16))) bf16_t Vt[HD * LDV];

    const int tid = threadIdx.x, lane = tid & 63, wave = tid >> 6;
    const int l15 = lane & 15, lg = lane >> 4;
    const int h = blockIdx.x, b = blockIdx.y;
    const bf16_t* Q = reinterpret_cast<const bf16_t*>(a.q);
    const bf16_t* K = reinterpret_cast<const bf16_t*>(a.k);
    const bf16_t* V = reinterpret_cast<const bf16_t*>(a.v);
    bf16_t* O = reinterpret_cast<bf16_t*>(a.out);
    const size_t base_row = (size_t)b * a.N;
    const int n = RAGGED ? a.ntok[b] : a.N;
    if constexpr (RAGGED) {
        for (int i = tid; i < (a.N - n) * 8; i += 256) {
            const int qr = n + (i >> 3);
            *reinterpret_cast<u32x4_t*>(O + (base_row + qr) * a.ldo + h * HD + (i & 7) * 8) = u32x4_t{0u, 0u, 0u, 0u};
        }
    }

#pragma unroll
    for (int it = 0; it < (NK * 8 + 255) / 256; ++it) {
        int idx = tid + it * 256;
        const bool ok = idx < NK * 8;
        idx = ok ? idx : NK * 8 - 1;
        const int key = idx >> 3, c = idx & 7;
        const int kr = key < n ? key : n - 1;
        const u32x4_t kc = *reinterpret_cast<const u32x4_t*>(K + (base_row + kr) * a.ldk + h * HD + c * 8);
        if (ok) *reinterpret_cast<u32x4_t*>(Ks + key * FA_LDK + c * 8) = kc;
    }
#pragma unroll
    for (int it = 0; it < (NB * 8 * 8 + 255) / 256; ++it) {
        int task = tid + it * 256;
        const bool ok = task < NB * 8 * 8;
        task = ok ? task : NB * 8 * 8 - 1;
        const int kg = task % (NB * 8), c = task / (NB * 8);
        u32x4_t vc[4];
#pragma unroll
        for (int e = 0; e < 4; ++e) {
            const int key = kg * 4 + e;
            const int kr = key < n ? key : n - 1;
            vc[e] = *reinterpret_cast<const u32x4_t*>(V + (base_row + kr) * a.ldv + h * HD + c * 8);
            if (key >= n) vc[e] = u32x4_t{0u, 0u, 0u, 0u};
        }
        if (ok) {
#pragma unroll
            for (int w = 0; w < 4; ++w) {
                uint2 even, odd;
                even.x = (vc[0][w] & 0xffffu) | (vc[1][w] << 16);
                even.y = (vc[2][w] & 0xffffu) | (vc[3][w] << 16);
                odd.x = (vc[0][w] >> 16) | (vc[1][w] & 0xffff0000u);
                odd.y = (vc[2][w] >> 16) | (vc[3][w] & 0xffff0000u);
                *reinterpret_cast<uint2*>(Vt + (c * 8 + 2 * w) * LDV + kg * 4) = even;
                *reinterpret_cast<uint2*>(Vt + (c * 8 + 2 * w + 1) * LDV + kg * 4) = odd;
            }
        }
    }
    __syncthreads();

    const int nqt = (n + 15) >> 4;
    const float c2 = a.scale * 1.4426950408889634f;

    auto process = [&](auto nt_c, int t0) {
        constexpr int NT = decltype(nt_c)::value;
        bf16x8_t qf[NT][2];
#pragma unroll
        for (int u = 0; u < NT; ++u) {
            int qr = (t0 + 4 * u) * 16 + l15;
            qr = qr < n ? qr : n - 1;
            const bf16_t* qp = Q + (base_row + qr) * a.ldq + h * HD + lg * 8;
            qf[u][0] = *reinterpret_cast<const bf16x8_t*>(qp);
            qf[u][1] = *reinterpret_cast<const bf16x8_t*>(qp + 32);
        }
        f32x4_t sacc[NT][NSUB];
#pragma unroll
        for (int st_ = 0; st_ < NSUB; ++st_) {
            const bf16x8_t kf0 = *reinterpret_cast<const bf16x8_t*>(Ks + (st_ * 16 + l15) * FA_LDK + lg * 8);
            const bf16x8_t kf1 = *reinterpret_cast<const bf16x8_t*>(Ks + (st_ * 16 + l15) * FA_LDK + 32 + lg * 8);
#pragma unroll
            for (int u = 0; u < NT; ++u) {
                sacc[u][st_] = mfma16(kf0, qf[u][0], f32x4_t{0.f, 0.f, 0.f, 0.f});
                sacc[u][st_] = mfma16(kf1, qf[u][1], sacc[u][st_]);
            }
            if constexpr (NSUB > 13) { if (st_ % 4 == 3) __builtin_amdgcn_sched_barrier(0); }
        }
        float inv_l[NT];
#pragma unroll
        for (int u = 0; u < NT; ++u) {
            if constexpr (RAGGED) {
#pragma unroll
                for (int st_ = 0; st_ < NSUB; ++st_)
#pragma unroll
                    for (int r = 0; r < 4; ++r)
                        if (st_ * 16 + lg * 4 + r >= n) sacc[u][st_][r] = -INFINITY;
            } else {
#pragma unroll
                for (int r = 0; r < 4; ++r)
                    if ((NSUB - 1) * 16 + lg * 4 + r >= a.N) sacc[u][NSUB - 1][r] = -INFINITY;
            }
            float m = -INFINITY;
#pragma unroll
            for (int st_ = 0; st_ < NSUB; ++st_)
#pragma unroll
                for (int r = 0; r < 4; ++r) m = fmaxf(m, sacc[u][st_][r]);
            m = fmaxf(m, __shfl_xor(m, 16, 64));
            m = fmaxf(m, __shfl_xor(m, 32, 64));
            const float mc = m * c2;
            float psum = 0.f;
#pragma unroll
            for (int st_ = 0; st_ < NSUB; ++st_)
#pragma unroll
                for (int r = 0; r < 4; ++r) {
                    const float p = __builtin_amdgcn_exp2f(sacc[u][st_][r] * c2 - mc);
                    sacc[u][st_][r] = p;
                    psum += p;
                }
            psum += __shfl_xor(psum, 16, 64);
            psum += __shfl_xor(psum, 32, 64);
            inv_l[u] = 1.0f / psum;
        }
        uint32_t pk2[NT][NSUB][2];
#pragma unroll
        for (int u = 0; u < NT; ++u)
#pragma unroll
            for (int st_ = 0; st_ < NSUB; ++st_) {
                pk2[u][st_][0] = pack2bf(sacc[u][st_][0], sacc[u][st_][1]);
                pk2[u][st_][1] = pack2bf(sacc[u][st_][2], sacc[u][st_][3]);
            }
        f32x4_t o_acc[NT][4];
#pragma unroll
        for (int u = 0; u < NT; ++u)
#pragma unroll
            for (int dt = 0; dt < 4; ++dt) o_acc[u][dt] = f32x4_t{0.f, 0.f, 0.f, 0.f};
#pragma unroll
        for (int blk = 0; blk < NB; ++blk) {
            bf16x8_t pf[NT];
#pragma unroll
            for (int u = 0; u < NT; ++u) {
                union { bf16x8_t v; uint32_t w[4]; } pk;
                pk.w[0] = pk2[u][2 * blk][0];
                pk.w[1] = pk2[u][2 * blk][1];
                const bool has1 = 2 * blk + 1 < NSUB;
                const int s1 = has1 ? 2 * blk + 1 : 0;
                pk.w[2] = has1 ? pk2[u][s1][0] : 0u;
                pk.w[3] = has1 ? pk2[u][s1][1] : 0u;
                pf[u] = pk.v;
            }
#pragma unroll
            for (int dt = 0; dt < 4; ++dt) {
                union { bf16x8_t v; uint2 h2[2]; } vf;
                const bf16_t* vp = Vt + (dt * 16 + l15) * LDV + blk * 32 + lg * 4;
                vf.h2[0] = *reinterpret_cast<const uint2*>(vp);
                vf.h2[1] = *reinterpret_cast<const uint2*>(vp + 16);
#pragma unroll
                for (int u = 0; u < NT; ++u)
                    o_acc[u][dt] = mfma16(vf.v, pf[u], o_acc[u][dt]);
            }
        }
#pragma unroll
        for (int u = 0; u < NT; ++u) {
            const int qr = (t0 + 4 * u) * 16 + l15;
            if (qr < n) {
                bf16_t* op = O + (base_row + qr) * a.ldo + h * HD;
#pragma unroll
                for (int dt = 0; dt < 4; ++dt) {
                    uint2 tt;
                    tt.x = pack2bf(o_acc[u][dt][0] * inv_l[u], o_acc[u][dt][1] * inv_l[u]);
                    tt.y = pack2bf(o_acc[u][dt][2] * inv_l[u], o_acc[u][dt][3] * inv_l[u]);
                    *reinterpret_cast<uint2*>(op + dt * 16 + lg * 4) = tt;
                }
            }
        }
    };

    for (int t0 = wave; t0 < nqt; t0 += 8) {
        if (t0 + 4 < nqt) process(std::integral_constant<int, 2>{}, t0);
        else process(std::integral_constant<int, 1>{}, t0);
    }
}

template <typename T>
__global__ void kv_repack_kernel(const T* __restrict__ qkv, T* __restrict__ kh, T* __restrict__ vh, int B, int N, int H,
                                 int d) {
    constexpr int CH = 16 / (int)sizeof(T);
    constexpr int CPH = HD / CH;
    const size_t per = (size_t)B * H * N * CPH;
    for (size_t i = blockIdx.x * (size_t)blockDim.x + threadIdx.x; i < 2 * per; i += (size_t)gridDim.x * blockDim.x) {
        const int kv = i >= per;
        size_t r = kv ? i - per : i;
        const int c = (int)(r % CPH); r /= CPH;
        const int n = (int)(r % N); r /= N;
        const int h = (int)(r % H);
        const int b = (int)(r / H);
        const T* src = qkv + ((size_t)b * N + n) * 3 * d + (kv ? 2 : 1) * d + h * HD + c * CH;
        T* dst = (kv ? vh : kh) + (((size_t)b * H + h) * N + n) * HD + c * CH;
        *reinterpret_cast<u32x4_t*>(dst) = *reinterpret_cast<const u32x4_t*>(src);
    }
}

template <typename T> struct Raw8;
template <> struct Raw8<bf16_t> {
    u32x4_t r;
    __device__ __forceinline__ void load(const bf16_t* p) { r = *reinterpret_cast<const u32x4_t*>(p); }
    __device__ __forceinline__ void load_nt(const bf16_t* p) { r = __builtin_nontemporal_load(reinterpret_cast<const u32x4_t*>(p)); }
    __device__ __forceinline__ void store(bf16_t* p) const { *reinterpret_cast<u32x4_t*>(p) = r; }
    __device__ __forceinline__ void zero() { r = u32x4_t{0u, 0u, 0u, 0u}; }
    __device__ __forceinline__ void get(float (&v)[8]) const {
#pragma unroll
        for (int i = 0; i < 4; ++i) {
            unpack2op(r[i], v[2 * i], v[2 * i + 1]);
        }
    }
};
template <> struct Raw8<float> {
    f32x4_t a, b;
    __device__ __forceinline__ void load(const float* p) {
        a = *reinterpret_cast<const f32x4_t*>(p);
        b = *reinterpret_cast<const f32x4_t*>(p + 4);
    }
    __device__ __forceinline__ void load_nt(const float* p) {
        a = __builtin_nontemporal_load(reinterpret_cast<const f32x4_t*>(p));
        b = __builtin_nontemporal_load(reinterpret_cast<const f32x4_t*>(p + 4));
    }
    __device__ __forceinline__ void store(float* p) const {
        *reinterpret_cast<f32x4_t*>(p) = a;
        *reinterpret_cast<f32x4_t*>(p + 4) = b;
    }
    __device__ __forceinline__ void zero() { a = f32x4_t{0.f, 0.f, 0.f, 0.f}; b = a; }
    __device__ __forceinline__ void get(float (&v)[8]) const {
#pragma unroll
        for (int i = 0; i < 4; ++i) { v[i] = a[i]; v[4 + i] = b[i]; }
    }
};

template <typename T, int KB, int PF = 8, int TI = 5>
__global__ __launch_bounds__(256) void attn_decode_kernel(AttnDecodeArgs a) {
    __shared__ float part[4][KB][HD + 2];

    const int tid = threadIdx.x;
    const int h = blockIdx.x, b = blockIdx.y, H = gridDim.x;
    const int k = a.beams;
    const T* QKV = reinterpret_cast<const T*>(a.qkv);
    const T* IMGK = reinterpret_cast<const T*>(a.img_k);
    const T* IMGV = reinterpret_cast<const T*>(a.img_v);
    T* TK = reinterpret_cast<T*>(a.txt_k);
    T* TV = reinterpret_cast<T*>(a.txt_v);
// ... 125 lines not shown
    }
    auto text_item = [&](int jj, const float (&kv)[8], const float (&vv)[8]) {
#pragma unroll
        for (int j = 0; j < KB; ++j) {
            if (j == jj) {
                const float sv = dot8(q[j], kv);
                const float mn = fmaxf(m[j], sv);
                const float al = fast_exp(m[j] - mn);
                const float p = fast_exp(sv - mn);
                l[j] = l[j] * al + p;
#pragma unroll
                for (int e = 0; e < 8; ++e) o[j][e] = o[j][e] * al + p * vv[e];
                m[j] = mn;
            }
        }
    };
#pragma unroll
    for (int u = 0; u < TI; ++u) {
        if (t_j[u] >= 0) {
            float kv[8], vv[8];
            tk[u].get(kv);
            tv[u].get(vv);
            text_item(t_j[u], kv, vv);
        }
    }
    for (int it = grp + 32 * TI; it < k * nt; it += 32) {
        const int j = it / nt, sidx = it % nt;
        float kv[8], vv[8];
        if (sidx == a.pos) {
            ld8(QKV + (size_t)(row0 + j) * ld3 + a.d + h * HD + sub * 8, kv);
            ld8(QKV + (size_t)(row0 + j) * ld3 + 2 * a.d + h * HD + sub * 8, vv);
        } else {
            const int srow = KB == 1 ? row0 : a.kv_src[(size_t)(row0 + j) * a.ld_src + sidx];
            ld8(TK + ((size_t)srow * a.T_max + sidx) * a.d + h * HD + sub * 8, kv);
            ld8(TV + ((size_t)srow * a.T_max + sidx) * a.d + h * HD + sub * 8, vv);
        }
        text_item(j, kv, vv);
    }

#pragma unroll
    for (int j = 0; j < KB; ++j) {
#pragma unroll
        for (int off = 8; off < 64; off <<= 1) {
            const float m2 = __shfl_xor(m[j], off, 64);
            const float l2 = __shfl_xor(l[j], off, 64);
            const float mn = fmaxf(m[j], m2);
            const float a1 = m[j] == -INFINITY ? 0.f : fast_exp(m[j] - mn);
            const float a2 = m2 == -INFINITY ? 0.f : fast_exp(m2 - mn);
            l[j] = l[j] * a1 + l2 * a2;
#pragma unroll
            for (int e = 0; e < 8; ++e) {
                const float o2 = __shfl_xor(o[j][e], off, 64);
                o[j][e] = o[j][e] * a1 + o2 * a2;
            }
            m[j] = mn;
        }
        if ((tid & 63) < 8 && j < k) {
#pragma unroll
            for (int e = 0; e < 8; ++e) part[wave][j][sub * 8 + e] = o[j][e];
            if (sub == 0) { part[wave][j][HD] = m[j]; part[wave][j][HD + 1] = l[j]; }
        }
    }
    __syncthreads();
    for (int i = tid; i < k * HD; i += 256) {
        const int j = i / HD, dd = i % HD;
        float mm = -INFINITY;
#pragma unroll
        for (int w = 0; w < 4; ++w) mm = fmaxf(mm, part[w][j][HD]);
        float num = 0.f, den = 0.f;
#pragma unroll
        for (int w = 0; w < 4; ++w) {
            const float mw = part[w][j][HD];
            const float aw = mw == -INFINITY ? 0.f : fast_exp(mw - mm);
            num += aw * part[w][j][dd];
            den += aw * part[w][j][HD + 1];
        }
        if constexpr (sizeof(T) == 2) {
            if (a.out_frag) { O[frag_offset(row0 + j, h * HD + dd, a.d >> 5)] = f2bf(num / den); continue; }
        }
        st<T>(O + (size_t)(row0 + j) * a.d + h * HD + dd, num / den);
    }
}

hipError_t launch_attn_full(const AttnFullArgs& a, int B, bool is_f32, int impl, hipStream_t s) {
    if (B <= 0 || a.N <= 0) return hipSuccess;
    if (impl == 1) {
        if (is_f32) return hipErrorInvalidValue;
        const int nsub = (a.N + 15) / 16;
        if (nsub == 13 && a.ntok) hipLaunchKernelGGL((attn_full_mfma_short_kernel<13, true>), dim3(a.H, B), dim3(256), 0, s, a);
        else if (nsub == 13) hipLaunchKernelGGL(attn_full_mfma_short_kernel<13>, dim3(a.H, B), dim3(256), 0, s, a);
        else if (nsub == 17 && a.ntok) hipLaunchKernelGGL((attn_full_mfma_short_kernel<17, true>), dim3(a.H, B), dim3(256), 0, s, a);
        else if (nsub == 17) hipLaunchKernelGGL(attn_full_mfma_short_kernel<17>, dim3(a.H, B), dim3(256), 0, s, a);
        else hipLaunchKernelGGL(attn_full_mfma_kernel, dim3((a.N + 255) / 256, a.H, B), dim3(256), 0, s, a);
    } else if (impl == 2) {
        if (is_f32) return hipErrorInvalidValue;
        hipLaunchKernelGGL(attn_full_mfma_kernel, dim3((a.N + 255) / 256, a.H, B), dim3(256), 0, s, a);
    } else if (is_f32) {
        hipLaunchKernelGGL(attn_full_valu_kernel<float>, dim3((a.N + 15) / 16, a.H, B), dim3(256), 0, s, a);
    } else {
        hipLaunchKernelGGL(attn_full_valu_kernel<bf16_t>, dim3((a.N + 15) / 16, a.H, B), dim3(256), 0, s, a);
    }
    return hipGetLastError();
}

hipError_t launch_kv_repack(const void* qkv, void* kh, void* vh, int B, int N, int H, int d, hipStream_t s) {
    if (B <= 0 || N <= 0) return hipSuccess;
    const size_t total = 2 * (size_t)B * H * N * 16;
    size_t grid = (total + 255) / 256;
    grid = grid > 8192 ? 8192 : grid;
    hipLaunchKernelGGL(kv_repack_kernel<float>, dim3((int)grid), dim3(256), 0, s, (const float*)qkv, (float*)kh, (float*)vh, B, N,
                       H, d);
    return hipGetLastError();
}

hipError_t launch_attn_decode(const AttnDecodeArgs& a, int B, int H, hipStream_t s) {
    if (B <= 0) return hipSuccess;
    if (a.beams > 8) return hipErrorInvalidValue;
    if (a.beams <= 1) hipLaunchKernelGGL((attn_decode_kernel<float, 1>), dim3(H, B), dim3(256), 0, s, a);
    else if (a.beams <= 2) hipLaunchKernelGGL((attn_decode_kernel<float, 2>), dim3(H, B), dim3(256), 0, s, a);
    else if (a.beams <= 4) hipLaunchKernelGGL((attn_decode_kernel<float, 4>), dim3(H, B), dim3(256), 0, s, a);
    else hipLaunchKernelGGL((attn_decode_kernel<float, 8>), dim3(H, B), dim3(256), 0, s, a);
    return hipGetLastError();
}

}
```

### generativeimage2text_amd/csrc/kernels_gemm.hip

```cpp
#include "gitmi_common.h"
#include "launchers.h"
#include <type_traits>

namespace gitmi {

template <typename TIn> struct GemmTraits;
template <> struct GemmTraits<bf16_t> {
    static constexpr int BK = 64;
    static constexpr int LDK = 72;
    static constexpr int CHUNK = 8;
};
template <> struct GemmTraits<float> {
    static constexpr int BK = 16;
    static constexpr int LDK = 20;
    static constexpr int CHUNK = 4;
};

__device__ __forceinline__ int xcd_remap(int b, int nwg) {
    const int q = nwg >> 3, r = nwg & 7;
    const int xcd = b & 7, idx = b >> 3;
    return (xcd < r ? xcd * (q + 1) : r * (q + 1) + (xcd - r) * q) + idx;
}

template <typename TOut>
// ... 185 lines not shown
#pragma unroll
                        for (int r = 0; r < 4; ++r) v[r] += t[r];
                    } else {
#pragma unroll
                        for (int r = 0; r < 4; ++r)
                            if (n + r < g.N) v[r] += (float)rp[r];
                    }
                } else {
                    const float* rp = g.res + (size_t)m * g.ldr + n;
                    if (full && vec_r) {
                        f32x4_t t = *reinterpret_cast<const f32x4_t*>(rp);
#pragma unroll
                        for (int r = 0; r < 4; ++r) v[r] += t[r];
                    } else {
#pragma unroll
                        for (int r = 0; r < 4; ++r)
                            if (n + r < g.N) v[r] += rp[r];
                    }
                }
            }
            TOut* cp = C + (size_t)m * g.ldc + n;
            if (full) {
                store4<TOut>(cp, v, vec_c);
            } else {
#pragma unroll
                for (int r = 0; r < 4; ++r)
                    if (n + r < g.N) st<TOut>(cp + r, v[r]);
            }
        }
    }
}

template <typename TIn, typename TOut, int BM, int BN>
static hipError_t launch_gemm_t(GemmArgs g, hipStream_t s) {
    const int tiles_m = (g.M + BM - 1) / BM;
    g.tiles_n = (g.N + BN - 1) / BN;
    g.nwg = tiles_m * g.tiles_n;
    hipLaunchKernelGGL((gemm_kernel<TIn, TOut, BM, BN>), dim3(g.nwg), dim3(256), 0, s, g);
    return hipGetLastError();
}

template <typename TIn, typename TOut>
static hipError_t launch_gemm_tiles(const GemmArgs& g, hipStream_t s) {
    if (g.M <= 64) return launch_gemm_t<TIn, TOut, 64, 64>(g, s);
    if (g.M <= 512 || (long)((g.M + 127) / 128) * ((g.N + 127) / 128) < 256)
        return launch_gemm_t<TIn, TOut, 64, 128>(g, s);
    return launch_gemm_t<TIn, TOut, 128, 128>(g, s);
}

static int g_gemm_impl = -1;
static int g_gemm_dbg = 0;
bool set_gemm_impl(int impl) {
    int dbg = 0;
    if (impl >= 0) { dbg = impl >> 8; impl &= 0xff; }
    if (impl != -1 && impl != 0 && impl != 9) return false;
    g_gemm_dbg = dbg;
    g_gemm_impl = impl;
    return true;
}

static bool gemm_fast_operands(const GemmArgs& g, bool in_f32, bool out_f32) {
    if (in_f32) return false;
    if (g.K % 64 != 0 || g.N % 8 != 0 || g.lda % 8 != 0) return false;
    if (g.ldc % (out_f32 ? 4 : 8) != 0) return false;
    if (g.res && g.ldr % (g.out_f16 ? 8 : 4) != 0) return false;
    if ((reinterpret_cast<uintptr_t>(g.A) | reinterpret_cast<uintptr_t>(g.W) | reinterpret_cast<uintptr_t>(g.C) |
         reinterpret_cast<uintptr_t>(g.res)) & 15)
        return false;
    return true;
}

bool gemm_uses_p8(const GemmArgs& g, bool in_f32, bool out_f32) {
    const bool fast_ok = g_gemm_impl != 0 && gemm_fast_operands(g, in_f32, out_f32) && gemm_p8_supports(g);
    return fast_ok && (g.M > 512 || g_gemm_impl == 9);
}

hipError_t launch_gemm(const GemmArgs& g_in, bool in_f32, bool out_f32, hipStream_t s) {
    GemmArgs g = g_in;
    g.dbg = g_gemm_dbg;
    if (g.M <= 0 || g.N <= 0) return hipSuccess;
    if (g.out_f16 && (in_f32 || out_f32 || g.K % 64 != 0)) return hipErrorInvalidValue;
    if (gemm_uses_p8(g, in_f32, out_f32)) return launch_gemm_p8(g, out_f32, s);
    if (g.ln_part || g.part_out || g.res_part) return hipErrorInvalidValue;
    if (g.out_f16) return launch_gemm_tiles<bf16_t, f16_t>(g, s);
    if (in_f32) {
        if (g.K % 16 != 0) return hipErrorInvalidValue;
        return out_f32 ? launch_gemm_tiles<float, float>(g, s) : launch_gemm_tiles<float, bf16_t>(g, s);
    }
    if (g.K % 64 != 0) return hipErrorInvalidValue;
    return out_f32 ? launch_gemm_tiles<bf16_t, float>(g, s) : launch_gemm_tiles<bf16_t, bf16_t>(g, s);
}

}
```

### generativeimage2text_amd/csrc/kernels_gemm10.hip

```cpp
#include "gitmi_common.h"
#include "launchers.h"
#include <type_traits>

namespace gitmi {

namespace {

constexpr int BN = 256, BK = 64;
constexpr int HALF_BYTES = 128 * BK * 2;
constexpr int BUF_BYTES = 4 * HALF_BYTES;
constexpr int LDS_BYTES = 2 * BUF_BYTES;
constexpr int SLOT_A0 = 0, SLOT_A1 = HALF_BYTES, SLOT_B0 = 2 * HALF_BYTES, SLOT_B1 = 3 * HALF_BYTES;

typedef __attribute__((address_space(3))) void lds_void_t;

#define P8_BARRIER()                           \
    do {                                       \
        __builtin_amdgcn_sched_barrier(0);     \
        __builtin_amdgcn_s_barrier();          \
        asm volatile("" ::: "memory");         \
        __builtin_amdgcn_sched_barrier(0);     \
    } while (0)

__device__ __forceinline__ float add_unfused(float a, float b) {
// ... 16 lines not shown
        "v_add_f32_dpp %0, %0, %0 row_ror:8 row_mask:0xf bank_mask:0xf\n\t"
        "v_add_f32_dpp %1, %1, %1 row_ror:8 row_mask:0xf bank_mask:0xf\n\t"
        "s_nop 0\n\t"
        "v_add_f32_dpp %0, %0, %0 row_bcast:15 row_mask:0xa bank_mask:0xf\n\t"
        "v_add_f32_dpp %1, %1, %1 row_bcast:15 row_mask:0xa bank_mask:0xf\n\t"
        "s_nop 1"
        : "+v"(a), "+v"(b));
}

#define P8_LDS_BARRIER()                                   \
    do {                                                   \
        asm volatile("s_waitcnt lgkmcnt(0)" ::: "memory"); \
        __builtin_amdgcn_s_barrier();                      \
        asm volatile("" ::: "memory");                     \
    } while (0)

template <typename T> __device__ __forceinline__ uint32_t pack2o(float lo, float hi) {
    if constexpr (std::is_same<T, f16_t>::value) return pack2h(lo, hi);
    else return pack2bf(lo, hi);
}
template <typename T> __device__ __forceinline__ void unpack2o(uint32_t u, float& lo, float& hi) {
    if constexpr (std::is_same<T, f16_t>::value) unpack2h(u, lo, hi);
    else unpack2op(u, lo, hi);
}

template <int N> __device__ __forceinline__ void wait_vm() {
    if constexpr (N == 8) asm volatile("s_waitcnt vmcnt(8)" ::: "memory");
    else if constexpr (N == 4) asm volatile("s_waitcnt vmcnt(4)" ::: "memory");
    else if constexpr (N == 2) asm volatile("s_waitcnt vmcnt(2)" ::: "memory");
    else if constexpr (N == 0) asm volatile("s_waitcnt vmcnt(0)" ::: "memory");
}

template <typename TOut, int ACT, int DBG = 0, int MH = 128, int EPI = 1, int MH1 = MH, int LNF = 0>
__global__ __launch_bounds__(512) void gemm_p8_kernel(GemmArgs g) {
    static_assert(LNF == 0 || sizeof(TOut) == 2, "LayerNorm folding: 16-bit outputs only");
    static_assert(MH % 32 == 0 && MH1 % 32 == 0 && MH1 <= MH && MH <= 128, "half tiles: multiples of 32 rows, second <= first");
    constexpr int BM = MH + MH1, MI = MH / 32, MI1 = MH1 / 32;
    __shared__ __attribute__((aligned(16))) unsigned char smem[LDS_BYTES];

    const int tid = threadIdx.x;
    const int lane = tid & 63;
    const int wave = __builtin_amdgcn_readfirstlane(tid >> 6);
    const int grp = wave >> 2, wc = wave & 3;
    const int l15 = lane & 15, lg = lane >> 4;
    uint64_t ts[8];
    auto stamp = [&](int i) {
        if constexpr ((DBG & 16) != 0) {
            __builtin_amdgcn_sched_barrier(0);
            ts[2 * i] = __builtin_amdgcn_s_memtime();
            ts[2 * i + 1] = __builtin_amdgcn_s_memrealtime();
            __builtin_amdgcn_sched_barrier(0);
        }
    };
    auto stamps_out = [&]() {
        if constexpr ((DBG & 16) != 0) {
            if (tid == 0) {
                uint64_t* o = reinterpret_cast<uint64_t*>(const_cast<float*>(g.res)) + (size_t)blockIdx.x * 8;
#pragma unroll
                for (int i = 0; i < 8; ++i) o[i] = ts[i];
            }
        }
    };
    stamp(0);

    int tile_m, tile_n;
    {
        const int x = blockIdx.x & 7, idx = blockIdx.x >> 3;
        const int ng = g.ng, mg = 8 / ng;
        const int gn = x % ng, gm = x / ng;
        const int tiles_m = (g.M + BM - 1) / BM;
        const int n_lo = gn * g.tiles_n / ng, n_hi = (gn + 1) * g.tiles_n / ng;
        const int nn = n_hi - n_lo;
        const int tg = tiles_m * nn;
        const int lo_t = gm * tg / mg, hi_t = (gm + 1) * tg / mg;
        if (idx >= hi_t - lo_t) return;
        const int L = lo_t + idx;
        tile_m = L / nn;
        tile_n = n_lo + L % nn;
    }
    const int m0 = tile_m * BM, n0 = tile_n * BN;

    const char* __restrict__ Ab = reinterpret_cast<const char*>(g.A);
    const char* __restrict__ Wb = reinterpret_cast<const char*>(g.W);

    const int Rl = lane >> 4, hi = (lane >> 3) & 1, lo = lane & 7;
    uint32_t a_off[2][2], w_off[2][2];
#pragma unroll
    for (int h = 0; h < 2; ++h)
#pragma unroll
        for (int q = 0; q < 2; ++q) {
            const int rr = h * MH + (wave * 2 + q) * 8 + 2 * Rl + (hi ^ q);
            const int ch = lo ^ (q * 4 + Rl);
            int m = m0 + rr;
            m = m < g.M ? m : g.M - 1;
            a_off[h][q] = ((uint32_t)m * (uint32_t)g.lda + ch * 8) * 2u;
            const int rn = h * 128 + (wave * 2 + q) * 8 + 2 * Rl + (hi ^ q);
            w_off[h][q] = ((uint32_t)(n0 + rn) * (uint32_t)g.K + ch * 8) * 2u;
        }
    auto issue = [&](int isw, int half, int kt) {
        if constexpr (DBG & 8) return;
        const char* src = (isw ? Wb : Ab) + (size_t)kt * (BK * 2);
        unsigned char* dst = smem + (kt & 1) * BUF_BYTES + (isw ? SLOT_B0 : SLOT_A0) + half * HALF_BYTES + wave * 2048;
        const uint32_t o0 = isw ? w_off[half][0] : a_off[half][0];
        const uint32_t o1 = isw ? w_off[half][1] : a_off[half][1];
        __builtin_amdgcn_global_load_lds((const void*)(src + o0), (lds_void_t*)(dst), 16, 0, 0);
        __builtin_amdgcn_global_load_lds((const void*)(src + o1), (lds_void_t*)(dst + 1024), 16, 0, 0);
    };

    const int rowpart = (l15 >> 1) * 256 + ((l15 & 1) ^ ((l15 >> 3) & 1)) * 128;
    const int x7 = (l15 >> 1) & 7;
    const int ch0 = ((0 * 4 + lg) ^ x7) * 16;
    const int ch1 = ((1 * 4 + lg) ^ x7) * 16;
    const int a_rd = grp * (MH / 2) * 128 + rowpart;
    const int a_rd1 = grp * (MH1 / 2) * 128 + rowpart + HALF_BYTES;
    const int w_rd = SLOT_B0 + wc * 32 * 128 + rowpart;

    f32x4_t acc[2][2][2][MI];

    bf16x8_t af[MI][2], wf0[2][2], wf1[2][2];

    auto read_a = [&](const unsigned char* sb, auto half_c) {
        if constexpr (DBG & 4) return;
        constexpr int half = decltype(half_c)::value;
        const int base = half ? a_rd1 : a_rd;
#pragma unroll
        for (int i = 0; i < (half ? MI1 : MI); ++i) {
            af[i][0] = *reinterpret_cast<const bf16x8_t*>(sb + base + i * 2048 + ch0);
            af[i][1] = *reinterpret_cast<const bf16x8_t*>(sb + base + i * 2048 + ch1);
        }
    };
    constexpr std::integral_constant<int, 0> H0{};
    constexpr std::integral_constant<int, 1> H1{};
    auto read_w = [&](const unsigned char* sb, int half, bf16x8_t (&wf)[2][2]) {
        if constexpr (DBG & 4) return;
#pragma unroll
        for (int j = 0; j < 2; ++j) {
            wf[j][0] = *reinterpret_cast<const bf16x8_t*>(sb + w_rd + half * HALF_BYTES + j * 2048 + ch0);
            wf[j][1] = *reinterpret_cast<const bf16x8_t*>(sb + w_rd + half * HALF_BYTES + j * 2048 + ch1);
        }
    };
    auto mma = [&](f32x4_t (&c)[2][MI], const bf16x8_t (&wf)[2][2], auto half_c) {
        if constexpr (DBG & 4) return;
        constexpr int MIq = decltype(half_c)::value ? MI1 : MI;
        __builtin_amdgcn_s_setprio(1);
#pragma unroll
        for (int kk = 0; kk < 2; ++kk)
#pragma unroll
            for (int j = 0; j < 2; ++j)
#pragma unroll
                for (int i = 0; i < MIq; ++i)
                    c[j][i] = mfma16(wf[j][kk], af[i][kk], c[j][i]);
        __builtin_amdgcn_s_setprio(0);
    };

    auto ktile = [&](auto mode_c, int t) {
        constexpr int MODE = decltype(mode_c)::value;
        const unsigned char* sb = smem + (t & 1) * BUF_BYTES;
        read_w(sb, 0, wf0);
        __builtin_amdgcn_sched_barrier(0);
        read_a(sb, H0);
        if constexpr (MODE <= 1) { issue(1, 1, t + 1); wait_vm<8>(); } else { wait_vm<2>(); }
        P8_BARRIER();
        mma(acc[0][0], wf0, H0);
        P8_BARRIER();
        read_w(sb, 1, wf1);
        if constexpr (MODE <= 1) { issue(0, 1, t + 1); wait_vm<8>(); } else { wait_vm<0>(); }
        P8_BARRIER();
        mma(acc[0][1], wf1, H0);
        P8_BARRIER();
        read_a(sb, H1);
        if constexpr (MODE == 0) { issue(0, 0, t + 2); wait_vm<8>(); }
        P8_BARRIER();
        mma(acc[1][1], wf1, H1);
        P8_BARRIER();
        if constexpr (MODE == 0) { issue(1, 0, t + 2); wait_vm<8>(); }
        else if constexpr (MODE == 1) { wait_vm<4>(); }
        P8_BARRIER();
        mma(acc[1][0], wf0, H1);
        P8_BARRIER();
    };

    float lmean[2][MI], lrstd[2][MI];
    unsigned char* const ln_lds = smem + BUF_BYTES + SLOT_A1;
    if constexpr (LNF == 1) {
// ... 95 lines not shown
    };

    if constexpr (sizeof(TOut) == 4 && EPI == 1) {
        float* Cf = reinterpret_cast<float*>(g.C);
        const float* R = g.res;
        const int col0 = n0 + wc * 32 + lg * 4;
        const bool has_res = R != nullptr && !(DBG & 1);
#pragma unroll
        for (int qm = 0; qm < 2; ++qm) {
            const int MIq = qm ? MI1 : MI, MHq = qm ? MH1 : MH;
            f32x4_t rr[MI][2][2];
            if (has_res) {
#pragma unroll
                for (int i = 0; i < MIq; ++i) {
                    const int m = m0 + qm * MH + grp * (MHq / 2) + i * 16 + l15;
                    const int mc = m < g.M ? m : g.M - 1;
                    const float* rp = R + (size_t)mc * g.ldr + col0;
#pragma unroll
                    for (int qn = 0; qn < 2; ++qn)
#pragma unroll
                        for (int j = 0; j < 2; ++j)
                            rr[i][qn][j] = *reinterpret_cast<const f32x4_t*>(rp + qn * 128 + j * 16);
                }
            }
#pragma unroll
            for (int i = 0; i < MIq; ++i) {
                const int m = m0 + qm * MH + grp * (MHq / 2) + i * 16 + l15;
                float* cp = Cf + (size_t)m * g.ldc + col0;
                const bool ok = m < g.M && !(DBG & 1);
#pragma unroll
                for (int qn = 0; qn < 2; ++qn)
#pragma unroll
                    for (int j = 0; j < 2; ++j) {
                        f32x4_t v;
#pragma unroll
                        for (int r = 0; r < 4; ++r) v[r] = apply_act_t<ACT>(acc[qm][qn][j][i][r] + bias4[qn][j][r]);
                        if (has_res) {
#pragma unroll
                            for (int r = 0; r < 4; ++r) v[r] = add_unfused(v[r], rr[i][qn][j][r]);
                        }
                        if (ok) *reinterpret_cast<f32x4_t*>(cp + qn * 128 + j * 16) = v;
                    }
            }
        }
        return;
    }

    float rgm[8], rbt[8];
    if constexpr (LNF == 2) {
        if (g.res_part) {
            ld8(g.res_gamma + n0 + (tid & 31) * 8, rgm);
            ld8(g.res_beta + n0 + (tid & 31) * 8, rbt);
        }
    }
#pragma unroll
    for (int qm = 0; qm < 2; ++qm)
#pragma unroll
        for (int s = 0; s < 2 / NQN; ++s) {
            const int MIq = qm ? MI1 : MI, MHq = qm ? MH1 : MH;
#pragma unroll
            for (int u = 0; u < NQN; ++u) {
                const int qn = s * NQN + u;
#pragma unroll
                for (int j = 0; j < 2; ++j) {
                    const int nl = u * 128 + wc * 32 + j * 16 + lg * 4;
#pragma unroll
                    for (int i = 0; i < MIq; ++i) {
                        float v[4];
#pragma unroll
                        for (int r = 0; r < 4; ++r) v[r] = apply_act_t<ACT>(ln_apply(acc[qm][qn][j][i][r], qm, qn, j, i, r) + bias4[qn][j][r]);
                        TOut* p = ep + (grp * (MHq / 2) + i * 16 + l15) * EPS + nl;
                        if constexpr (sizeof(TOut) == 4) {
                            *reinterpret_cast<f32x4_t*>(p) = f32x4_t{v[0], v[1], v[2], v[3]};
                        } else {
                            uint2 t2;
                            t2.x = pack2o<TOut>(v[0], v[1]);
                            t2.y = pack2o<TOut>(v[2], v[3]);
                            *reinterpret_cast<uint2*>(p) = t2;
                        }
                    }
                }
            }
            P8_LDS_BARRIER();
#pragma unroll 4
            for (int q = 0; q < MHq * CPR / 512; ++q) {
                const int chunk = tid + q * 512;
                const int row = chunk / CPR, cc = chunk % CPR;
                const int m = m0 + qm * MH + row;
                const int n = n0 + s * WCOL + cc * EPC;
                if (m < g.M && !(DBG & 1)) {
                    if constexpr (sizeof(TOut) == 4) {
                        f32x4_t v = *reinterpret_cast<const f32x4_t*>(ep + row * EPS + cc * EPC);
                        if (g.res && !(DBG & 16)) {
                            const f32x4_t rr = *reinterpret_cast<const f32x4_t*>(g.res + (size_t)m * g.ldr + n);
                            v[0] += rr[0]; v[1] += rr[1]; v[2] += rr[2]; v[3] += rr[3];
                        }
                        *reinterpret_cast<f32x4_t*>(C + (size_t)m * g.ldc + n) = v;
                    } else if constexpr (LNF == 2) {
                    } else {
                        u32x4_t v = *reinterpret_cast<const u32x4_t*>(ep + row * EPS + cc * EPC);
                        if (g.res && !(DBG & 16)) {
                            float f[8], rs[8];
#pragma unroll
                            for (int e = 0; e < 4; ++e) unpack2o<TOut>(v[e], f[2 * e], f[2 * e + 1]);
                            if constexpr (std::is_same<TOut, f16_t>::value) {
                                const u32x4_t rr = *reinterpret_cast<const u32x4_t*>(reinterpret_cast<const f16_t*>(g.res) + (size_t)m * g.ldr + n);
#pragma unroll
                                for (int e = 0; e < 4; ++e) unpack2h(rr[e], rs[2 * e], rs[2 * e + 1]);
                            } else {
                                const float* rp = g.res + (size_t)m * g.ldr + n;
                                const f32x4_t r0 = *reinterpret_cast<const f32x4_t*>(rp);
                                const f32x4_t r1 = *reinterpret_cast<const f32x4_t*>(rp + 4);
#pragma unroll
                                for (int e = 0; e < 4; ++e) { rs[e] = r0[e]; rs[4 + e] = r1[e]; }
                            }
#pragma unroll
                            for (int e = 0; e < 8; ++e) f[e] += rs[e];
#pragma unroll
                            for (int e = 0; e < 4; ++e) v[e] = pack2o<TOut>(f[2 * e], f[2 * e + 1]);
                        }
                        TOut* cp = C + (size_t)m * g.ldc + n;
                        if (g.dbg & 512)
                            *reinterpret_cast<u32x4_t*>(cp) = v;
                        else
                            asm volatile("global_store_dwordx4 %0, %1, off sc1\n\ts_nop 1" ::"v"(cp), "v"(v) : "memory");
                    }
                }
                if constexpr (LNF == 2) {
                    static_assert(LNF != 2 || CPR == 32, "one stream row per half wave");
                    const bool ok = m < g.M;
                    const int mc = ok ? m : g.M - 1;
                    u32x4_t v = *reinterpret_cast<const u32x4_t*>(ep + row * EPS + cc * EPC);
                    float f[8];
#pragma unroll
                    for (int e = 0; e < 4; ++e) unpack2h(v[e], f[2 * e], f[2 * e + 1]);
                    if (g.res) {
                        float rs[8];
                        const u32x4_t rr = *reinterpret_cast<const u32x4_t*>(reinterpret_cast<const f16_t*>(g.res) + (size_t)mc * g.ldr + n);
#pragma unroll
                        for (int e = 0; e < 4; ++e) unpack2h(rr[e], rs[2 * e], rs[2 * e + 1]);
                        if (g.res_part) {
                            const f32x4_t* pp = reinterpret_cast<const f32x4_t*>(g.res_part + (size_t)mc * 4);
                            const f32x4_t p0 = pp[0], p1 = pp[1];
                            const float mean = ((p0[0] + p0[2]) + (p1[0] + p1[2])) * g.res_inv_d;
                            const float rstd = rsqrtf(fmaxf(((p0[1] + p0[3]) + (p1[1] + p1[3])) * g.res_inv_d - mean * mean, 0.f) + g.res_eps);
#pragma unroll
                            for (int e = 0; e < 8; ++e) rs[e] = fmaf((rs[e] - mean) * rstd, rgm[e], rbt[e]);
                        }
#pragma unroll
                        for (int e = 0; e < 8; ++e) f[e] += rs[e];
#pragma unroll
                        for (int e = 0; e < 4; ++e) v[e] = pack2h(f[2 * e], f[2 * e + 1]);
                    }
                    if (g.part_out) {
                        typedef __attribute__((ext_vector_type(2))) float f32x2_t;
                        f32x2_t s2 = {0.f, 0.f}, q2 = {0.f, 0.f};
#pragma unroll
                        for (int e = 0; e < 4; ++e) {
                            float x0, x1;
                            unpack2h(v[e], x0, x1);
                            const f32x2_t x = {x0, x1};
                            s2 += x;
                            q2 = __builtin_elementwise_fma(x, x, q2);
                        }
                        float sx = s2[0] + s2[1], sq = q2[0] + q2[1];
                        half_wave_sum2_hi(sx, sq);
                        if (ok && cc == 16 && !(DBG & 1)) g.part_out[(size_t)m * 4 + tile_n] = float2{sx, sq};
                    }
                    if (ok && !(DBG & 1)) {
                        TOut* cp = C + (size_t)m * g.ldc + n;
                        asm volatile("global_store_dwordx4 %0, %1, off sc1\n\ts_nop 1" ::"v"(cp), "v"(v) : "memory");
                    }
                }
            }
            P8_LDS_BARRIER();
        }
    if constexpr ((DBG & 16) != 0) {
        asm volatile("s_waitcnt vmcnt(0)" ::: "memory");
        stamp(3);
        stamps_out();
    }
}

}

template <typename TOut, int MH, int EPI = 1, int MH1 = MH, int LNF = 0>
static void launch_p8_t(const GemmArgs& g, hipStream_t s) {
    if constexpr (LNF == 2) {
        hipLaunchKernelGGL((gemm_p8_kernel<TOut, GITMI_ACT_NONE, 0, MH, EPI, MH1, LNF>), dim3(g.nwg), dim3(512), 0, s, g);
        return;
    } else {
    if (g.dbg && LNF == 0) {
        if constexpr (MH == 128 && MH1 == 128) {
            switch (g.dbg) {
                case 1: hipLaunchKernelGGL((gemm_p8_kernel<TOut, 0, 1>), dim3(g.nwg), dim3(512), 0, s, g); return;
                case 2: hipLaunchKernelGGL((gemm_p8_kernel<TOut, 0, 2>), dim3(g.nwg), dim3(512), 0, s, g); return;
                case 6: hipLaunchKernelGGL((gemm_p8_kernel<TOut, 0, 6>), dim3(g.nwg), dim3(512), 0, s, g); return;
                case 10: hipLaunchKernelGGL((gemm_p8_kernel<TOut, 0, 10>), dim3(g.nwg), dim3(512), 0, s, g); return;
#ifdef GITMI_PROBE
                case 16: hipLaunchKernelGGL((gemm_p8_kernel<TOut, 0, 16>), dim3(g.nwg), dim3(512), 0, s, g); return;
                case 17: hipLaunchKernelGGL((gemm_p8_kernel<TOut, 0, 17>), dim3(g.nwg), dim3(512), 0, s, g); return;
                case 18: hipLaunchKernelGGL((gemm_p8_kernel<TOut, 0, 18>), dim3(g.nwg), dim3(512), 0, s, g); return;
                case 22: hipLaunchKernelGGL((gemm_p8_kernel<TOut, 0, 22>), dim3(g.nwg), dim3(512), 0, s, g); return;
                case 26: hipLaunchKernelGGL((gemm_p8_kernel<TOut, 0, 26>), dim3(g.nwg), dim3(512), 0, s, g); return;
#endif
                default: break;
            }
        }
    }
    switch (g.act) {
        case GITMI_ACT_QUICKGELU:
            hipLaunchKernelGGL((gemm_p8_kernel<TOut, GITMI_ACT_QUICKGELU, 0, MH, EPI, MH1, LNF>), dim3(g.nwg), dim3(512), 0, s, g); break;
        case GITMI_ACT_GELU_ERF:
            hipLaunchKernelGGL((gemm_p8_kernel<TOut, GITMI_ACT_GELU_ERF, 0, MH, EPI, MH1, LNF>), dim3(g.nwg), dim3(512), 0, s, g); break;
        default:
            hipLaunchKernelGGL((gemm_p8_kernel<TOut, GITMI_ACT_NONE, 0, MH, EPI, MH1, LNF>), dim3(g.nwg), dim3(512), 0, s, g); break;
    }
    }
}

bool gemm_p8_supports(const GemmArgs& g) {
    return g.K % BK == 0 && g.K >= 2 * BK && g.N % BN == 0 &&
           (double)g.M * g.lda * 2.0 < 4.0e9 && (double)g.N * g.K * 2.0 < 4.0e9;
}

static int p8_xcd_count(const GemmArgs& g, int bm, int ng, int* max_nn_out) {
    const int tiles_m = (g.M + bm - 1) / bm, tiles_n = g.N / BN, mg = 8 / ng;
    int max_cnt = 0, max_nn = 0;
    for (int x = 0; x < 8; ++x) {
        const int gn = x % ng, gm = x / ng;
        const int nn = (gn + 1) * tiles_n / ng - gn * tiles_n / ng;
        const int tg = tiles_m * nn;
        const int cnt = (gm + 1) * tg / mg - gm * tg / mg;
        max_cnt = cnt > max_cnt ? cnt : max_cnt;
        max_nn = nn > max_nn ? nn : max_nn;
    }
    if (max_nn_out) *max_nn_out = max_nn;
    return max_cnt;
}
static int p8_plan(const GemmArgs& g, int bm, int* ng_out, int* max_cnt_out) {
    const int tiles_n = g.N / BN;
    int best_ng = 1, best_rounds = 1 << 30, best_cnt = 0, best_panels = 1 << 30;
    for (int ng = 1; ng <= 8 && ng <= tiles_n; ng *= 2) {
        int max_nn = 0;
        const int max_cnt = p8_xcd_count(g, bm, ng, &max_nn);
        const int rounds = (max_cnt + 31) / 32;
        const int panels = (32 + max_nn - 1) / max_nn + (max_nn < 32 ? max_nn : 32);
        if (rounds < best_rounds || (rounds == best_rounds && panels < best_panels)) {
            best_ng = ng; best_rounds = rounds; best_cnt = max_cnt; best_panels = panels;
        }
    }
    if (ng_out) *ng_out = best_ng;
    if (max_cnt_out) *max_cnt_out = best_cnt;
    return best_rounds;
}

int gemm_p8_cost(const GemmArgs& g, int bm) {
    const int rounds = p8_plan(g, bm, nullptr, nullptr);
    const int ktile = 1450 * (90 + 166 * bm / 256) / 256;
    return rounds * (1450 + (g.K / BK) * ktile + 4700 * bm / 256);
}

template <int MH, int MH1>
static void launch_p8_height(const GemmArgs& g, bool out_f32, bool staged, hipStream_t s) {
#ifdef GITMI_OPS_F16
    if (g.ln_part) { launch_p8_t<bf16_t, MH, 1, MH1, 1>(g, s); return; }
    if (g.part_out || g.res_part) { launch_p8_t<f16_t, MH, 1, MH1, 2>(g, s); return; }
#endif
    if (g.out_f16) launch_p8_t<f16_t, MH, 1, MH1>(g, s);
    else if (!out_f32) launch_p8_t<bf16_t, MH, 1, MH1>(g, s);
    else if (staged) launch_p8_t<float, MH, 0, MH1>(g, s);
    else launch_p8_t<float, MH, 1, MH1>(g, s);
}

hipError_t launch_gemm_p8(GemmArgs g, bool out_f32, hipStream_t s) {
    if (g.ln_part || g.part_out || g.res_part) {
#ifndef GITMI_OPS_F16
        return hipErrorInvalidValue;
#endif
        if (g.ln_part && (out_f32 || g.out_f16 || g.res || !g.ln_colsum || g.ln_nparts < 1 || g.part_out || g.res_part)) return hipErrorInvalidValue;
        if ((g.part_out || g.res_part) && (!g.out_f16 || out_f32 || g.act != 0 || g.N > 1024)) return hipErrorInvalidValue;
        if (g.res_part && (!g.res || !g.res_gamma || !g.res_beta || g.res_nparts < 1)) return hipErrorInvalidValue;
    }
    static const int heights[5] = {256, 224, 192, 160, 128};
    int bm = 256;
    if (!g.shared) {
        int best = gemm_p8_cost(g, 256);
        for (int h = 1; h < 5; ++h) {
            const int c = gemm_p8_cost(g, heights[h]);
            if (c < best) { best = c; bm = heights[h]; }
        }
    }
    if (g.dbg & 64) bm = 192;
    if (g.dbg & 128) bm = 256;
    if (g.dbg & 16384) bm = 160;
    if (g.dbg & 32768) bm = 224;
    if (g.dbg & 65536) bm = 128;
    g.dbg &= ~(64 | 128 | 16384 | 32768 | 65536);
    g.tiles_n = g.N / BN;
    int max_cnt = 0;
    p8_plan(g, bm, &g.ng, &max_cnt);
    if (g.dbg & (1024 | 2048 | 4096 | 8192)) {
        const int ng = (g.dbg & 1024) ? 1 : (g.dbg & 2048) ? 2 : (g.dbg & 4096) ? 4 : 8;
        g.dbg &= ~(1024 | 2048 | 4096 | 8192);
        if (ng <= g.tiles_n) { g.ng = ng; max_cnt = p8_xcd_count(g, bm, ng, nullptr); }
    }
    g.nwg = 8 * max_cnt;
    const bool staged = (g.dbg & 256) != 0;
    g.dbg &= ~256;
    switch (bm) {
        case 224: launch_p8_height<128, 96>(g, out_f32, staged, s); break;
        case 192: launch_p8_height<96, 96>(g, out_f32, staged, s); break;
        case 160: launch_p8_height<96, 64>(g, out_f32, staged, s); break;
        case 128: launch_p8_height<64, 64>(g, out_f32, staged, s); break;
        default: launch_p8_height<128, 128>(g, out_f32, staged, s); break;
    }
    return hipGetLastError();
}

}
```

### generativeimage2text_amd/csrc/launchers.h

```cpp
#pragma once
#include <hip/hip_runtime.h>
#include <stddef.h>

namespace gitmi {

struct GemmArgs {
    const void* A; const void* W; const float* bias; const float* res; void* C;
    int M, N, K;
    int lda, ldc, ldr;
    int act;
    int tiles_n, nwg;
    int ng;
    int dbg;
    int out_f16;
    int shared;
    const float2* ln_part; int ln_nparts; const float* ln_colsum; float ln_inv_d, ln_eps;
    float2* part_out;
    const float2* res_part; int res_nparts; const float* res_gamma; const float* res_beta; float res_inv_d, res_eps;
};
bool gemm_uses_p8(const GemmArgs& g, bool in_f32, bool out_f32);
hipError_t launch_gemm(const GemmArgs& g, bool in_f32, bool out_f32, hipStream_t s);
hipError_t launch_gemm_p8(GemmArgs g, bool out_f32, hipStream_t s);
bool gemm_p8_supports(const GemmArgs& g);
int gemm_p8_cost(const GemmArgs& g, int bm);
bool set_gemm_impl(int impl);

struct DGemmArgs {
    const unsigned short* A; const unsigned short* W;
    const float* bias;
    const float* colsum;
    const float2* stats_in;
    int strips_in; float inv_d, eps_in;
    void* C;
    int c_frag;
    const float* res_x;
    const float2* res_stats; int res_strips; const float* res_gamma; const float* res_beta; float res_inv_d, res_eps;
    float* x_out; unsigned short* xb_out; float2* stats_out;
    int M, N, K, lda, ldc, act;
    int dbg;
    int rows_per_wg;
    int strips_per_wg;
    int no_row_walk;
};
hipError_t launch_dgemm(const DGemmArgs& g, hipStream_t s);
struct DLn { const float2* stats; int strips; float inv_d, eps; const float* gamma; const float* beta; };
inline DGemmArgs dgemm_ln(const void* A, const void* W, const float* bias, const float* colsum, const DLn* ln, void* C, int c_frag,
                          int act, int M, int N, int K) {
    DGemmArgs g{};
    g.A = (const unsigned short*)A; g.lda = K; g.W = (const unsigned short*)W; g.bias = bias;
    if (ln) { g.colsum = colsum; g.stats_in = ln->stats; g.strips_in = ln->strips; g.inv_d = ln->inv_d; g.eps_in = ln->eps; }
    g.C = C; g.ldc = N; g.c_frag = c_frag; g.act = act; g.M = M; g.N = N; g.K = K;
    return g;
}
inline DGemmArgs dgemm_to_stream(const void* A, const void* W, const float* bias, const float* res_x, const DLn* res_ln, float* x_out,
                                 void* xb_out, float2* stats_out, int M, int N, int K) {
    DGemmArgs g{};
    g.A = (const unsigned short*)A; g.lda = K; g.W = (const unsigned short*)W; g.bias = bias; g.res_x = res_x;
    if (res_ln) {
        g.res_stats = res_ln->stats; g.res_strips = res_ln->strips; g.res_gamma = res_ln->gamma; g.res_beta = res_ln->beta;
        g.res_inv_d = res_ln->inv_d; g.res_eps = res_ln->eps;
    }
    g.x_out = x_out; g.xb_out = (unsigned short*)xb_out; g.stats_out = stats_out; g.M = M; g.N = N; g.K = K;
    return g;
}

struct BanArgs {
    const unsigned int* words; const int* set_of; const int* min_new; const int* ngram;
    int W, eos;
};

struct VocabArgs {
    const unsigned short* A; int lda; const unsigned short* W; const float* bias; const float* colsum;
    const float2* stats_in; int strips_in; float inv_d, eps_in;
    int M, N, K, cols_per_wg;
    const int* ids; int ld_ids, cur_len; const int* plen; int beams, suppress_kind;
    float rep_penalty;
    float* part_val; int* part_idx; float2* part_lse;
    float* logits_out; int ld_logits;
    int max_wgs;
    int nblk;
    BanArgs ban;
};
hipError_t launch_vocab_topm(const VocabArgs& g, int mtop, hipStream_t s);
int vocab_parts(int V, int cols_per_wg);
int vocab_mtop_slots(int mtop);

hipError_t launch_layernorm(const float* x, int ldx, const float* gamma, const float* beta, float eps,
                            const float* add_after, void* y_t, int ld_t, bool t_is_f32, float* y_f, int ld_f,
                            int rows, int D, int map_n_in, int map_n_out, int map_off, hipStream_t s);
hipError_t launch_im2col(const float* img, void* out, bool out_f32, int B, int H, int W, int p, int K, int Kpad,
                         hipStream_t s);
hipError_t launch_pos_bicubic(const float* pos, float* out, int g, int gh, int gw, int D, hipStream_t s);
hipError_t launch_ragged_stage(const float* src, float* dst, size_t slot, int4* meta, int* ntok, int B, int p, size_t max_pixels,
                               int Nmax, hipStream_t s);
hipError_t launch_im2col_ragged(const float* stage, size_t slot, const int4* meta, void* out, bool out_f32, int B, int Nmax,
                                int p, int K, int Kpad, hipStream_t s);
hipError_t launch_vit_assemble_ragged(const float* patch_out, const float* cls, const float* pos, int g, const int4* meta,
                                      const float* gamma, const float* beta, float eps, void* X, bool x_f16, int B, int Nmax,
                                      int p, int D, float2* part, hipStream_t s);
hipError_t launch_zero_pad_rows(void* x, bool is_f32, int ld, const int* ntok, int B, int Nmax, hipStream_t s);
hipError_t launch_ragged_report(const int4* meta, const int* image_of, int Q, int nout_per, float* logprob, int* info,
                                int* bad, hipStream_t s);
hipError_t launch_vit_assemble_ln(const float* patch_out, const float* cls, const float* pos, const float* gamma,
                                  const float* beta, float eps, void* X, bool x_f16, int B, int N, int D, float2* part,
                                  int nparts, hipStream_t s);
hipError_t launch_layernorm_s16(const void* x, int ldx, const float* gamma, const float* beta, float eps,
                                const float* add_after, void* y_t, int ld_t, bool t_is_f32, void* y_s, int ld_s,
                                int rows, int D, int map_n_in, int map_n_out, int map_off, hipStream_t s);
hipError_t launch_embed_ln(const int* ids, int ld_ids, int pos, const float* words, const float* positions,
                           const float* gamma, const float* beta, float eps, float* h_f, void* h_t, bool t_is_f32,
                           int R, int D, int vocab, bool frag, hipStream_t s);
hipError_t launch_context_embed(const long long* tokens, int ld, const int4* seg, int Q, const int* cnt, const float* words,
                                const float* positions, const float* gamma, const float* beta, float eps, void* feats, bool t_is_f32,
                                float* feats_f, int* ntok, int B, int n_img, int stride, int D, int vocab, int max_pos, hipStream_t s);
hipError_t launch_frag_pack(const void* src_bf16, void* dst_bf16, int rows, int rows_out, int K, hipStream_t s);
hipError_t launch_convert_pad(const float* src, void* dst, bool dst_f32, size_t rows, int K, int Kpad,
                              hipStream_t s);
hipError_t launch_convert(const void* src, bool src_f32, void* dst, bool dst_f32, size_t n, hipStream_t s);
hipError_t launch_chain_input(const float* x, void* xb_frag, float2* stats, int R, int d, hipStream_t s);
hipError_t launch_copy_f32(const float* src, int lds, float* dst, int ldd, int rows, int cols, hipStream_t s);
hipError_t launch_fill_i32(int* dst, int value, int n, hipStream_t s);

constexpr int MEMORY_MAX_LAYERS = 31;
constexpr int MEMORY_HEADER_BYTES = 256, MEMORY_HEADER_WORDS = 16;
constexpr int MEMORY_MAGIC = 0x4d495447;
enum { MEMW_MAGIC = 0, MEMW_VERSION = 1, MEMW_FP0 = 2, MEMW_FP_END = 9, MEMW_N = 9, MEMW_IMG_ROWS = 10, MEMW_CTX_ROWS = 11,
       MEMW_F = 12, MEMW_H = 13, MEMW_W = 14, MEMW_REJECTED = 15 };
struct MemoryEntry {
    int image, slot, n, rsv;
    int hdr[MEMORY_HEADER_WORDS + 4];
};
struct MemoryArgs {
    void* feats;
    void* kv[MEMORY_MAX_LAYERS];
    int layers, stride;
    int feat_row, kv_row, kv_ld, kv_col;
    size_t slot_bytes, feat_plane, kv_plane;
    int* ntok; int4* meta;
};
hipError_t launch_memory_pack(const MemoryArgs& a, void* store, const MemoryEntry* tab, int entries, int max_n, hipStream_t s);
hipError_t launch_memory_unpack(const MemoryArgs& a, const void* store, const MemoryEntry* tab, int entries, hipStream_t s);

struct FeaturePiece { int image, dst0, src0, rows; const float* temb; };
struct FeatureArgs {
    void* feats;
    const void* src;
    const FeaturePiece* pieces; int pieces_n;
    const int* count;
    int stride, D;
    int* ntok; int4* meta;
};
hipError_t launch_feature_install(const FeatureArgs& a, int B, bool src16, bool dst16, hipStream_t s);

struct AttnFullArgs {
    const void* q; const void* k; const void* v; void* out;
    int ldq, ldk, ldv, ldo;
    int N, H;
    float scale;
    const int* ntok;
};
hipError_t launch_attn_full(const AttnFullArgs& a, int B, bool is_f32, int impl, hipStream_t s);

struct AttnDecodeArgs {
    const void* qkv; const void* img_k; const void* img_v; void* txt_k; void* txt_v; void* out;
    const int* kv_src;
    const int* img_of;
    int ld_src;
    int d;
    int N_img, T_max, pos, beams;
    int N_pad;
    int out_frag;
    float scale;
    int dbg;
    int pairs_per_wg;
    int stream_wgs;
    int waves_per_pair;
    int n_pairs;
    const int* ntok;
    const unsigned short* x; const unsigned short* w; const float* bias; const float* colsum;
    const float2* stats_in; int strips_in; float inv_d, eps_in;
    int M;
};
hipError_t launch_kv_repack(const void* qkv, void* kh, void* vh, int B, int N, int H, int d, hipStream_t s);
hipError_t launch_attn_decode(const AttnDecodeArgs& a, int B, int H, hipStream_t s);
hipError_t launch_kv_repack_frag(const void* qkv, void* kf, void* vt, int B, int N, int N_pad, int H, int d, hipStream_t s);
hipError_t launch_attn_decode_mfma(const AttnDecodeArgs& a, int B, int H, hipStream_t s);
int attn_decode_pairs_per_wg(const AttnDecodeArgs& a, int B, int H);
bool attn_decode_qkv_form(const AttnDecodeArgs& a, int B, int H);
inline void attn_decode_set_qkv(AttnDecodeArgs& a, const DGemmArgs& g) {
    a.x = g.A; a.w = g.W; a.bias = g.bias; a.colsum = g.colsum;
    a.stats_in = g.stats_in; a.strips_in = g.strips_in; a.inv_d = g.inv_d; a.eps_in = g.eps_in; a.M = g.M;
}
hipError_t launch_attn_decode_qkv(const AttnDecodeArgs& a, int B, int H, hipStream_t s);

constexpr int SS_NHMAX = 8;
struct SearchState {
    int B, k, pn, T, V, eos, kind;
    int prefixed;
    int sampled;
    double length_penalty;
    double* len_norm;
    const long long* start;
    int ld_start;
    const int* plen;
    int* ids[2];
    int* kv_src[2];
    float* score[2];
    int* done;
    int nh;
    int* hyp_n;
    int* hyp_cnt;
    double* hyp_worst;
    double* hyp_score;
    int* hyp_len;
    int* hyp_seq;
    int* hyp_tok;
    int* stop;
    int* early;
    int* info;
};
struct StepCands {
    const float* part_val; const int* part_idx; const float2* part_lse;
    int nparts, slots;
};
struct EmbedArgs {
    const float* words; const float* positions; const float* gamma; const float* beta; float eps;
    float* h_f; void* h_t; int D, vocab;
    int frag;
};
int row_topm_slots(int M);
hipError_t launch_sample_rows(const float* logits, int ldl, int V, int R, float temperature, int top_k, float top_p,
                              int ndraw, unsigned long long seed, int step, float* part_val, int* part_idx,
                              float2* part_lse, float* filtered_out, const int* ids, int ld_ids, int cur_len,
                              float rep_penalty, int stride, hipStream_t s,
                              const BanArgs* ban = nullptr, const int* plen = nullptr, int beams = 1);
struct TrieArgs {
    const int* child_off; const int* child_tok; const int* child_node;
    int* cursor;
};
hipError_t launch_trie_select(const float* logits, int ldl, int V, const int* ids, int ld_ids, int cur_len, const int* plen,
                              int eos, const TrieArgs& tr, int B, float* part_val, int* part_idx, float2* part_lse,
                              hipStream_t s);
hipError_t launch_row_topm(const float* logits, int ldl, int V, const int* ids, int ld_ids, int cur_len,
                           const int* plen, int beams, int suppress_kind, float rep_penalty, int M, int R,
// ... 54 lines not shown
```

### generativeimage2text_amd/engine.py

```python
from __future__ import annotations

import ctypes as C
import os
from typing import Dict, List, Mapping, Optional, Sequence, Tuple

import torch

_HERE = os.path.dirname(os.path.abspath(__file__))
LIB_PATH = os.path.join(_HERE, "libgitmi.so")
LIB_PATH_F16 = os.path.join(_HERE, "libgitmi_f16.so")
LIB_PATH_EXP = os.path.join(_HERE, "libgitmi_exp.so")
LIB_PATH_F16_EXP = os.path.join(_HERE, "libgitmi_f16_exp.so")

PREC_BF16, PREC_F32 = 0, 1
DTYPE_F32, DTYPE_BF16, DTYPE_F16 = 0, 1, 2
DTYPE_F16_STREAM = 3
SEARCH_AUTOREGRESSIVE, SEARCH_GENERATOR, SEARCH_TRIE = 0, 1, 2
SEARCH_SCORE = 3
SEARCH_ATTEND = 4
SEARCH_CONTEXT = 5
SEARCH_TREE_SCORE = 6
SEARCH_KEEP = 7
SEARCH_RECALL = 8
SEARCH_FEATURES = 9
# ... 1090 lines not shown
    f32 = lambda t: t.to(device=feats.device, dtype=torch.float32).contiguous()
    words, positions, gamma, beta = f32(words), f32(positions), f32(gamma), f32(beta)
    ntok = torch.full((B,), -1, dtype=torch.int32, device=feats.device)
    copy = torch.zeros(B, stride, D, dtype=torch.float32, device=feats.device) if want_f32 else None
    lens, img = _sentence_tables([int(v) for v in lengths], image_of)
    _ck(fn(tokens.data_ptr(), ld, lens, img, Q, words.data_ptr(), int(words.shape[0]), positions.data_ptr(), int(positions.shape[0]),
           gamma.data_ptr(), beta.data_ptr(), float(eps), feats.data_ptr(), _torch_dtype_code(feats), _ptr(copy), ntok.data_ptr(),
           B, int(n_img), stride, D, _stream()), lib)
    return ntok, copy


def op_gemm(A: torch.Tensor, W: torch.Tensor, bias: Optional[torch.Tensor] = None,
            residual: Optional[torch.Tensor] = None, act: int = ACT_NONE,
            out_dtype: torch.dtype = torch.float32, stream_rows: bool = False) -> torch.Tensor:
    assert A.is_cuda and W.is_cuda and A.dtype == W.dtype and A.is_contiguous() and W.is_contiguous()
    M, K = A.shape
    N = W.shape[0]
    if stream_rows:
        if A.dtype == torch.float32:
            raise GitmiError("op_gemm: fp16 stream rows need 16-bit operands")
        if residual is not None and (residual.dtype != torch.float16 or residual.shape != (M, N) or not residual.is_contiguous()):
            raise GitmiError("op_gemm: the stream form's residual is contiguous fp16 [M, N] rows")
        lib, out_code, out_dtype = _op_library(A.dtype), DTYPE_F16_STREAM, torch.float16
    else:
        if residual is not None and residual.dtype != torch.float32:
            raise GitmiError("op_gemm: the residual is fp32 (fp16 rows: stream_rows=True)")
        lib = _op_library(A.dtype, out_dtype, fp32_ok=True)
        out_code = {torch.float32: DTYPE_F32, torch.bfloat16: DTYPE_BF16, torch.float16: DTYPE_F16}[out_dtype]
    out = torch.empty(M, N, device=A.device, dtype=out_dtype)
    _ck(lib.gitmi_op_gemm(A.data_ptr(), W.data_ptr(), _ptr(bias), _ptr(residual), out.data_ptr(), M, N, K, K, N,
                          _torch_dtype_code(A), out_code, act, _stream()), lib)
    return out


def op_gemm_ln(A: torch.Tensor, W: torch.Tensor, bias: Optional[torch.Tensor], *, colsum: Optional[torch.Tensor] = None,
               ln_part: Optional[torch.Tensor] = None, ln_eps: float = 1e-5, residual: Optional[torch.Tensor] = None,
               res_part: Optional[torch.Tensor] = None, res_gamma: Optional[torch.Tensor] = None,
               res_beta: Optional[torch.Tensor] = None, res_eps: float = 1e-12, want_part: bool = False, act: int = ACT_NONE):
    lib = load_library("f16")
    assert A.dtype == torch.float16 and W.dtype == torch.float16 and A.is_contiguous() and W.is_contiguous()
    M, K = A.shape
    N = W.shape[0]
    out = torch.empty(M, N, device=A.device, dtype=torch.float16)
    part = torch.zeros(M, 4, 2, device=A.device, dtype=torch.float32) if want_part else None
    _ck(lib.gitmi_op_gemm_ln(A.data_ptr(), W.data_ptr(), _ptr(bias), _ptr(colsum), _ptr(ln_part), ln_eps, _ptr(residual),
                             _ptr(res_part), _ptr(res_gamma), _ptr(res_beta), res_eps, out.data_ptr(), _ptr(part), M, N, K, act,
                             _stream()), lib)
    return (out, part) if want_part else out


def op_gemm_form(A: torch.Tensor, W: torch.Tensor, C: torch.Tensor, M: int, N: int, K: int, *, lda: Optional[int] = None,
                 ldc: Optional[int] = None, bias=None, res=None, ldr: int = 0, act: int = ACT_NONE, stream_rows: bool = False,
                 shared: bool = False, ln_part=None, colsum=None, ln_eps: float = 1e-5, part_out=None, res_part=None,
                 res_gamma=None, res_beta=None, res_eps: float = 1e-5, operands: Optional[str] = None) -> None:
    if A.dtype != W.dtype:
        raise GitmiError(f"operands must share one type, got {A.dtype} / {W.dtype}")
    lib = _exp_library(A.dtype, *(() if stream_rows else (C.dtype,)), operands=operands)
    out_code = DTYPE_F16_STREAM if stream_rows else _torch_dtype_code(C)
    _ck(_experiment_only(lib, "gitmi_debug_gemm_form")(
        A.data_ptr(), int(K if lda is None else lda), W.data_ptr(), _ptr(bias), _ptr(res), int(ldr), C.data_ptr(),
        int(N if ldc is None else ldc), int(M), int(N), int(K), int(act), _torch_dtype_code(A), out_code, int(bool(shared)),
        _ptr(ln_part), _ptr(colsum), float(ln_eps), _ptr(part_out), _ptr(res_part), _ptr(res_gamma), _ptr(res_beta), float(res_eps),
        _stream()), lib)


def op_layernorm(x: torch.Tensor, gamma: torch.Tensor, beta: torch.Tensor, eps: float,
                 out_dtype: torch.dtype = torch.float32) -> torch.Tensor:
    lib = _op_library(out_dtype, fp32_ok=True)
    rows, D = x.shape
    out = torch.empty(rows, D, device=x.device, dtype=out_dtype)
    _ck(lib.gitmi_op_layernorm(x.data_ptr(), gamma.data_ptr(), beta.data_ptr(), eps, out.data_ptr(), None, rows, D,
                               _torch_dtype_code(out), _stream()), lib)
    return out


def op_attention(qkv: torch.Tensor, B: int, N: int, H: int, impl: int) -> torch.Tensor:
    lib = _op_library(qkv.dtype, fp32_ok=True)
    assert qkv.is_cuda and qkv.is_contiguous() and qkv.shape == (B * N, 3 * H * 64)
    out = torch.empty(B * N, H * 64, device=qkv.device, dtype=qkv.dtype)
    _ck(lib.gitmi_op_attention(qkv.data_ptr(), out.data_ptr(), B, N, H, _torch_dtype_code(qkv), impl, _stream()), lib)
    return out


def strip_stats(x: torch.Tensor) -> torch.Tensor:
    M, N = x.shape
    xs = x.float().reshape(M, N // 16, 16)
    return torch.stack([xs.sum(-1), (xs * xs).sum(-1)], dim=-1).permute(1, 0, 2).contiguous()


def to_frag(x: torch.Tensor, row_multiple: int = 16) -> torch.Tensor:
    R, K = x.shape
    Rp = (R + row_multiple - 1) // row_multiple * row_multiple
    xp = torch.zeros(Rp, K, dtype=x.dtype, device=x.device)
    xp[:R] = x
    return xp.reshape(Rp // 16, 16, K // 32, 4, 8).permute(0, 2, 3, 1, 4).contiguous().reshape(Rp, K)


def from_frag(xf: torch.Tensor, rows: int) -> torch.Tensor:
    Rp, K = xf.shape
    return xf.reshape(Rp // 16, K // 32, 4, 16, 8).permute(0, 3, 1, 2, 4).reshape(Rp, K)[:rows].contiguous()


def _pad_vec(v: Optional[torch.Tensor], n: int) -> Optional[torch.Tensor]:
    if v is None:
        return None
    out = torch.zeros(n, dtype=v.dtype, device=v.device)
    out[:v.numel()] = v
    return out


def op_dgemm(A: torch.Tensor, W: torch.Tensor, bias: torch.Tensor, colsum: Optional[torch.Tensor] = None,
             stats: Optional[torch.Tensor] = None, eps: float = 1e-12, act: int = ACT_NONE,
             frag_out: bool = False, packed: bool = False, strips_per_wg: int = 0) -> torch.Tensor:
    lib = _op_library(A.dtype, W.dtype)
    if packed:
        Af, Wf, M, N, K = A, W, int(A.shape[0]), int(bias.numel()), int(A.shape[1])
        if stats is not None:
            M = int(stats.shape[1])
    else:
        M, K = A.shape
        N = W.shape[0]
        Af, Wf = to_frag(A, 64), to_frag(W)
    out = torch.empty((M + 15) // 16 * 16 if frag_out else M, N, device=A.device, dtype=A.dtype)
    strips = 0 if stats is None else int(stats.shape[0])
    _ck(lib.gitmi_op_dgemm(Af.data_ptr(), Wf.data_ptr(), bias.data_ptr(), _ptr(colsum), _ptr(stats), strips, eps,
                           out.data_ptr(), 1 if frag_out else 0, M, N, K, act, int(strips_per_wg), _stream()), lib)
    return from_frag(out, M) if (frag_out and not packed) else out


def op_dgemm_res(A: torch.Tensor, W: torch.Tensor, bias: torch.Tensor, res_x: torch.Tensor,
                 res_stats: Optional[torch.Tensor] = None, res_gamma: Optional[torch.Tensor] = None,
                 res_beta: Optional[torch.Tensor] = None, res_eps: float = 1e-12, packed: bool = False):
    lib = _op_library(A.dtype, W.dtype)
    M, N = res_x.shape
    K = A.shape[1]
    Af, Wf = (A, W) if packed else (to_frag(A, 64), to_frag(W))
    x = torch.empty(M, N, device=A.device, dtype=torch.float32)
    xb = torch.empty((M + 15) // 16 * 16, (N + 31) // 32 * 32, device=A.device, dtype=A.dtype)
    st = torch.empty(N // 16, M, 2, device=A.device, dtype=torch.float32)
    strips = 0 if res_stats is None else int(res_stats.shape[0])
    _ck(lib.gitmi_op_dgemm_res(Af.data_ptr(), Wf.data_ptr(), bias.data_ptr(), res_x.data_ptr(), _ptr(res_stats), strips,
                               _ptr(res_gamma), _ptr(res_beta), res_eps, x.data_ptr(), xb.data_ptr(), st.data_ptr(),
                               M, N, K, _stream()), lib)
    return x, (xb if packed else from_frag(xb, M)[:, :N].contiguous()), st


def op_dgemm_form(A: torch.Tensor, W: torch.Tensor, bias: torch.Tensor, M: Optional[int] = None, *, colsum=None, stats=None,
                  eps: float = 1e-12, act: int = ACT_NONE, frag_out: bool = False, out: Optional[torch.Tensor] = None,
                  res_x=None, res_stats=None, res_gamma=None, res_beta=None, res_eps: float = 1e-12, x=None, xb=None,
                  stats_out=None, packed: bool = False, rows_per_wg: int = 0, strips_per_wg: int = 0, no_row_walk: int = 0):
    lib = _exp_library(A.dtype, W.dtype)
    own = A.dtype
    if own == torch.float32:
        raise GitmiError(f"operands must be bf16 or fp16, got {A.dtype} / {W.dtype}")
    if packed:
        if M is None:
            raise ValueError("packed operands: M is required")
        Af, Wf = A, W
    else:
        M = int(A.shape[0]) if M is None else int(M)
        Af, Wf = to_frag(A, 64), to_frag(W)
    M, N, K = int(M), int(bias.numel()), int(A.shape[1])
    Mp = (M + 15) // 16 * 16
    producer = res_x is not None
    if producer:
        x = torch.empty(M, N, device=A.device, dtype=torch.float32) if x is None else x
# ... 411 lines not shown
```

Baseline: 11780 captions/s.

## Write QKV in head-blocked layout from GEMM epilogue and read it blocked in attention

The QKV projection GEMM epilogue now writes its output per image and head as contiguous [tokens x 64] blocks. The single-pass attention kernel reads Q/K/V and writes the context in that blocked layout through per-image and per-head strides. The output projection GEMM then reads the blocked context via magic-number division in its A addressing. The aim is contiguous, coalesced per-head tiles for attention in both the ViT encoder and the decoder image prefill, in place of strided row reads. The cost is extra integer address math in the GEMM load and store paths, a new p_q buffer, and a path limited to impl 1 with 193..208 or 257..272 tokens and no ragged batches.

```diff
diff --git a/generativeimage2text_amd/csrc/abi_ops.hip b/generativeimage2text_amd/csrc/abi_ops.hip
--- a/generativeimage2text_amd/csrc/abi_ops.hip
+++ b/generativeimage2text_amd/csrc/abi_ops.hip
@@ -25,6 +25,20 @@
     return fail("%s: %s is %s (%d), but this library's 16-bit operands are %s (libgitmi%s.so)", op, arg, dtype_name(dtype), dtype,
                 dtype_name(gitmi_operand_dtype()), gitmi_operand_dtype() == GITMI_DTYPE_F16 ? "_f16" : "");
 }
+
+struct OpBlocked { int tokens = 0, cols = 0, a = 0; };
+#ifdef GITMI_EXPERIMENT
+#include <stdio.h>
+#include <stdlib.h>
+static OpBlocked op_blocked() {
+    OpBlocked b;
+    if (const char* env = getenv("GITMI_OP_BLOCKED"))
+        if (sscanf(env, "%d,%d,%d", &b.tokens, &b.cols, &b.a) != 3) b.tokens = -1;
+    return b;
+}
+#else
+static OpBlocked op_blocked() { return OpBlocked(); }
+#endif
 
 extern "C" int gitmi_op_gemm(const void* A, const void* W, const float* bias, const float* residual, void* C, int M,
                              int N, int K, int lda, int ldc, int in_dtype, int out_dtype, int act, void* stream) {
@@ -81,6 +95,14 @@
     RCK(check_dtype("op_attention", "dtype", dtype));
     const size_t esz = dtype == GITMI_DTYPE_F32 ? 4 : 2;
     const int D = H * 64;
+    if (const OpBlocked ob = op_blocked(); ob.tokens) {
+        if (ob.tokens != N || (ob.cols != 3 * D && ob.cols != D)) return fail("op_attention: GITMI_OP_BLOCKED does not describe this call");
+        const void* rows = ob.cols == D ? qkv : nullptr;
+        const void* q = rows ? (const char*)qkv + (size_t)B * N * 3 * D * esz : qkv;
+        if (launch_attn_full(attn_full_blocked_args(q, rows, out, D, H, N), B, dtype == GITMI_DTYPE_F32, impl, (hipStream_t)stream) != hipSuccess)
+            return fail("op_attention: blocked operands are served by the single-pass 16-bit kernel only (impl 1, 193..208 or 257..272 rows)");
+        return 0;
+    }
     AttnFullArgs a{};
     a.q = qkv;
     a.k = (const char*)qkv + (size_t)D * esz;
@@ -342,6 +364,13 @@
         }
         if (!gemm_uses_p8(g, false, false))
             return fail("debug_gemm_form: the folded forms exist in gemm_p8_kernel only (more than 512 rows, N %% 256 == 0, K >= 128, 16-byte aligned rows)");
+    }
+    if (const OpBlocked ob = op_blocked(); ob.tokens) {
+        g.blk_tokens = ob.tokens; g.blk_cols = ob.cols; g.a_blk = ob.a ? 1 : 0;
+        if (ob.cols) g.Cb = (char*)C + (size_t)M * ldc * 2;
+        if (!gemm_uses_p8(g, in_f32, out_f32) || !gemm_p8_blocked_ok(g, out_f32))
+            return fail("debug_gemm_form: GITMI_OP_BLOCKED=%d,%d,%d does not describe a launch gemm_p8_kernel has the blocked forms for", ob.tokens,
+                        ob.cols, ob.a);
     }
     HIPCK(launch_gemm(g, in_f32, out_f32, (hipStream_t)stream));
     return 0;
diff --git a/generativeimage2text_amd/csrc/engine.hip b/generativeimage2text_amd/csrc/engine.hip
--- a/generativeimage2text_amd/csrc/engine.hip
+++ b/generativeimage2text_amd/csrc/engine.hip
@@ -85,14 +85,19 @@
 static void stream_written(Stream& st, const float2* part, const float* gamma, const float* beta, float eps) {
     st.part = part; st.gamma = gamma; st.beta = beta; st.eps = eps;
 }
+struct BlockedOut { int tokens = 0, cols = 0; void* Cb = nullptr; };
+static void set_blocked_out(GemmArgs& g, const BlockedOut* blk) {
+    if (blk) { g.blk_tokens = blk->tokens; g.blk_cols = blk->cols; g.Cb = blk->Cb; }
+}
 static int ln_gemm(gitmi_engine* e, hipStream_t s, const Stream& st, const Folded& f, const void* W, const float* bias, void* C,
-                   int ldc, int col0, int N, int act) {
+                   int ldc, int col0, int N, int act, const BlockedOut* blk = nullptr) {
     const int D = st.D;
     const size_t woff = (size_t)col0 * D * e->pol.esz;
     C = (char*)C + (size_t)col0 * e->pol.esz;
     if (st.fold) {
         GemmArgs g = gemm_args(st.x, D, (const char*)f.w + woff, f.bias + col0, nullptr, 0, C, ldc, st.M, N, D, act);
         g.ln_part = st.part; g.ln_nparts = D / 256; g.ln_colsum = f.colsum + col0; g.ln_inv_d = 1.0f / (float)D; g.ln_eps = st.eps;
+        set_blocked_out(g, blk);
         return gemm_run(e, s, g, false, false, st.tag);
     }
     if (e->pol.stream_f16)
@@ -100,15 +105,18 @@
     else
         HIPCK(launch_layernorm((const float*)st.x, D, st.gamma, st.beta, st.eps, nullptr, st.t, D, e->pol.f32, st.xn, st.xn ? D : 0, st.M,
                                D, 0, 0, 0, s));
-    return gemm(e, s, st.t, D, (const char*)W + woff, bias + col0, nullptr, 0, C, ldc, e->pol.f32, st.M, N, D, act, st.tag);
+    GemmArgs g = gemm_args(st.t, D, (const char*)W + woff, bias + col0, nullptr, 0, C, ldc, st.M, N, D, act);
+    set_blocked_out(g, blk);
+    return gemm_run(e, s, g, e->pol.f32, e->pol.f32, st.tag);
 }
 static int gemm_to_stream(gitmi_engine* e, hipStream_t s, Stream& st, const void* A, int lda, const void* W, const float* bias, int K,
-                          bool residual, const float* gamma, const float* beta, float eps) {
+                          bool residual, const float* gamma, const float* beta, float eps, int a_tokens = 0) {
     const int D = st.D;
     float2* part = gamma ? stream_part_out(st) : nullptr;
     const void* res = !residual ? nullptr : st.xn && !st.fold ? st.xn : st.x;
     GemmArgs g = gemm_args(A, lda, W, bias, res, residual ? D : 0, st.x, D, st.M, D, K, 0);
     g.out_f16 = e->pol.stream_f16 ? 1 : 0;
+    if (a_tokens > 0) { g.a_blk = 1; g.blk_tokens = a_tokens; }
     if (st.fold) {
         g.part_out = part;
         if (residual && st.xn) {
@@ -132,6 +140,11 @@
     a.N = N; a.H = heads; a.scale = 0.125f;
     a.ntok = ntok;
     HIPCK(launch_attn_full(a, batch, e->pol.f32, e->pol.attn_impl, s));
+    return 0;
+}
+static int attn_full_blocked(gitmi_engine* e, const void* q, const void* kv_rows, void* out, int width, int heads, int N, int batch,
+                             hipStream_t s) {
+    HIPCK(launch_attn_full(attn_full_blocked_args(q, kv_rows, out, width, heads, N), batch, false, e->pol.attn_impl, s));
     return 0;
 }
 static int dec_layer_tail(gitmi_engine* e, hipStream_t s, const DecLayerW& L, const void* ctx, float* hf, void* ht, float* y, void* u,
@@ -192,6 +205,7 @@
 #endif
 #ifdef GITMI_EXPERIMENT
     if (const char* env = getenv("GITMI_ATTN_IMPL")) e->pol.attn_impl = e->pol.f32 ? 0 : atoi(env);
+    if (const char* env = getenv("GITMI_ATTN_BLOCKED")) e->pol.attn_blocked = atoi(env) != 0;
     if (const char* env = getenv("GITMI_GRAPH")) e->pol.use_graph = atoi(env) != 0;
     if (const char* env = getenv("GITMI_ATTN_DBG")) e->pol.attn_dbg = atoi(env);
     if (const char* env = getenv("GITMI_ATTN_PW")) e->pol.attn_pw = atoi(env);
@@ -315,6 +329,18 @@
               on_p8(e->v_u, 4 * D, L.w2, e->v_x, D, M, D, 4 * D, true);
     if (st.fold) st.parts[0] = st.parts[1] = e->v_part;
     return st;
+}
+static bool attn_blocked(const gitmi_engine* e, const Stream& x, const void* wqkv, const void* qkv, const void* ctx, const void* wo,
+                         int tokens, const int* ntok) {
+    const int M = x.M, w = x.D;
+    if (!e->pol.attn_blocked || e->pol.f32 || ntok || e->pol.attn_impl != 1 || !attn_full_short_form(tokens)) return false;
+    if (w % 256 || M % tokens) return false;
+    GemmArgs g = gemm_args(x.fold ? x.x : x.t, w, wqkv, nullptr, nullptr, 0, const_cast<void*>(qkv), 3 * w, M, 3 * w, w, 0);
+    g.blk_tokens = tokens; g.blk_cols = w; g.Cb = const_cast<void*>(qkv);
+    if (!gemm_uses_p8(g, false, false) || !gemm_p8_blocked_ok(g, false)) return false;
+    g = gemm_args(ctx, w, wo, nullptr, nullptr, 0, x.x, w, M, w, w, 0);
+    g.out_f16 = e->pol.stream_f16 ? 1 : 0; g.a_blk = 1; g.blk_tokens = tokens;
+    return gemm_uses_p8(g, false, !e->pol.stream_f16) && gemm_p8_blocked_ok(g, !e->pol.stream_f16);
 }
 static Stream prefill_stream(gitmi_engine* e, int M) {
     const int d = e->cfg.dec_hidden, ffn = e->cfg.dec_ffn, D = e->cfg.vit_width;
@@ -359,12 +385,16 @@
     HIPCK(launch_vit_assemble_ln(e->patch_out, e->w.cls, e->pos_cur, e->w.lnpre_g, e->w.lnpre_b, 1e-5f, e->v_x, e->pol.stream_f16, BI, N, D,
                                  part, D / 256, s));
     stream_written(x, part, e->w.vit[0].ln1g, e->w.vit[0].ln1b, 1e-5f);
+    const int* ntok = e->ragged ? e->rg_ntok : nullptr;
+    const bool blocked = attn_blocked(e, x, x.fold ? e->w.vit[0].qkv_f.w : e->w.vit[0].wqkv, e->v_qkv, e->v_ctx, e->w.vit[0].wo, N, ntok);
+    const BlockedOut qkv_blk{N, 3 * D, e->v_qkv};
     for (int l = 0; l < c.vit_layers; ++l) {
         const VitLayerW& L = e->w.vit[l];
         const VitLayerW* Ln = l + 1 < c.vit_layers ? &e->w.vit[l + 1] : nullptr;
-        RCK(ln_gemm(e, s, x, L.qkv_f, L.wqkv, L.bqkv, e->v_qkv, 3 * D, 0, 3 * D, 0));
-        RCK(attn_full_packed(e, e->v_qkv, e->v_ctx, D, c.vit_heads, N, BI, e->ragged ? e->rg_ntok : nullptr, s));
-        RCK(gemm_to_stream(e, s, x, e->v_ctx, D, L.wo, L.bo, D, true, L.ln2g, L.ln2b, 1e-5f));
+        RCK(ln_gemm(e, s, x, L.qkv_f, L.wqkv, L.bqkv, e->v_qkv, 3 * D, 0, 3 * D, 0, blocked ? &qkv_blk : nullptr));
+        if (blocked) RCK(attn_full_blocked(e, e->v_qkv, nullptr, e->v_ctx, D, c.vit_heads, N, BI, s));
+        else RCK(attn_full_packed(e, e->v_qkv, e->v_ctx, D, c.vit_heads, N, BI, ntok, s));
+        RCK(gemm_to_stream(e, s, x, e->v_ctx, D, L.wo, L.bo, D, true, L.ln2g, L.ln2b, 1e-5f, blocked ? N : 0));
         RCK(ln_gemm(e, s, x, L.ffn1_f, L.w1, L.b1, e->v_u, 4 * D, 0, 4 * D, 1));
         RCK(gemm_to_stream(e, s, x, e->v_u, 4 * D, L.w2, L.b2, 4 * D, true, Ln ? Ln->ln1g : nullptr, Ln ? Ln->ln1b : nullptr, 1e-5f));
     }
@@ -408,15 +438,19 @@
     SpanGuard phase(e, s, TAG_PREFILL, 0);
     Stream y = prefill_stream(e, M);
     RCK(gemm_to_stream(e, s, y, e->feats, D, e->w.vp_w, e->w.vp_b, D, false, e->w.vp_lng, e->w.vp_lnb, 1e-5f));
+    const bool blocked = c.dec_layers > 1 && attn_blocked(e, y, y.fold ? e->w.dec[0].qkv_pf.w : e->w.dec[0].wqkv, e->img_kv[0], e->p_ctx,
+                                                          e->w.dec[0].wo, Nimg, key_counts(e));
+    const BlockedOut q_blk{Nimg, d, e->p_q};
     for (int l = 0; l < c.dec_layers; ++l) {
         const DecLayerW& L = e->w.dec[l];
         const bool last = l + 1 == c.dec_layers;
         const int col0 = last ? d : 0;
-        RCK(ln_gemm(e, s, y, L.qkv_pf, L.wqkv, L.bqkv, e->img_kv[l], 3 * d, col0, 3 * d - col0, 0));
+        RCK(ln_gemm(e, s, y, L.qkv_pf, L.wqkv, L.bqkv, e->img_kv[l], 3 * d, col0, 3 * d - col0, 0, blocked && !last ? &q_blk : nullptr));
         RCK(kv_repack(e, l, B, Nimg, s));
         if (last) break;
-        RCK(attn_full_packed(e, e->img_kv[l], e->p_ctx, d, c.dec_heads, Nimg, B, key_counts(e), s));
-        RCK(gemm_to_stream(e, s, y, e->p_ctx, d, L.wo, L.bo, d, true, L.lnag, L.lnab, 1e-12f));
+        if (blocked) RCK(attn_full_blocked(e, e->p_q, e->img_kv[l], e->p_ctx, d, c.dec_heads, Nimg, B, s));
+        else RCK(attn_full_packed(e, e->img_kv[l], e->p_ctx, d, c.dec_heads, Nimg, B, key_counts(e), s));
+        RCK(gemm_to_stream(e, s, y, e->p_ctx, d, L.wo, L.bo, d, true, L.lnag, L.lnab, 1e-12f, blocked ? Nimg : 0));
         RCK(ln_gemm(e, s, y, L.ffn1_pf, L.w1, L.b1, e->p_u, ffn, 0, ffn, 2));
         RCK(gemm_to_stream(e, s, y, e->p_u, ffn, L.w2, L.b2, ffn, true, L.lnog, L.lnob, 1e-12f));
     }
diff --git a/generativeimage2text_amd/csrc/engine_state.h b/generativeimage2text_amd/csrc/engine_state.h
--- a/generativeimage2text_amd/csrc/engine_state.h
+++ b/generativeimage2text_amd/csrc/engine_state.h
@@ -98,6 +98,7 @@
     bool stream_f16 = false;
     bool ln_fold = false;
     bool ln_fold_ready = false;
+    bool attn_blocked = true;
     bool skinny = true;
     bool use_graph = true;
     bool use_temb = true;
@@ -152,6 +153,7 @@
     void* feats = nullptr;
     float *p_y = nullptr, *p_hf = nullptr;
     void *p_ht = nullptr, *p_ctx = nullptr, *p_u = nullptr;
+    void* p_q = nullptr;
     std::vector<void*> img_kv;
     std::vector<void*> img_kh, img_vh;
     float *d_y = nullptr, *d_hf = nullptr, *logits = nullptr;
diff --git a/generativeimage2text_amd/csrc/engine_weights.hip b/generativeimage2text_amd/csrc/engine_weights.hip
--- a/generativeimage2text_amd/csrc/engine_weights.hip
+++ b/generativeimage2text_amd/csrc/engine_weights.hip
@@ -147,6 +147,7 @@
     RCK(dev_alloc_t(e, &e->p_hf, Mp * d));
     RCK(dev_alloc(e, &e->p_ht, Mp * d * esz));
     RCK(dev_alloc(e, &e->p_ctx, Mp * d * esz));
+    if (!e->pol.f32) RCK(dev_alloc(e, &e->p_q, Mp * d * esz));
     RCK(dev_alloc(e, &e->p_u, Mp * c.dec_ffn * esz));
     e->img_kv.resize(c.dec_layers);
     e->img_kh.resize(c.dec_layers);
diff --git a/generativeimage2text_amd/csrc/kernels_attn.hip b/generativeimage2text_amd/csrc/kernels_attn.hip
--- a/generativeimage2text_amd/csrc/kernels_attn.hip
+++ b/generativeimage2text_amd/csrc/kernels_attn.hip
@@ -237,16 +237,15 @@
     const int tid = threadIdx.x, lane = tid & 63, wave = tid >> 6;
     const int l15 = lane & 15, lg = lane >> 4;
     const int h = blockIdx.x, b = blockIdx.y;
-    const bf16_t* Q = reinterpret_cast<const bf16_t*>(a.q);
-    const bf16_t* K = reinterpret_cast<const bf16_t*>(a.k);
-    const bf16_t* V = reinterpret_cast<const bf16_t*>(a.v);
-    bf16_t* O = reinterpret_cast<bf16_t*>(a.out);
-    const size_t base_row = (size_t)b * a.N;
+    const bf16_t* Q = reinterpret_cast<const bf16_t*>(a.q) + (size_t)b * a.is_q + (size_t)h * a.hs_q;
+    const bf16_t* K = reinterpret_cast<const bf16_t*>(a.k) + (size_t)b * a.is_k + (size_t)h * a.hs_k;
+    const bf16_t* V = reinterpret_cast<const bf16_t*>(a.v) + (size_t)b * a.is_v + (size_t)h * a.hs_v;
+    bf16_t* O = reinterpret_cast<bf16_t*>(a.out) + (size_t)b * a.is_o + (size_t)h * a.hs_o;
     const int n = RAGGED ? a.ntok[b] : a.N;
     if constexpr (RAGGED) {
         for (int i = tid; i < (a.N - n) * 8; i += 256) {
             const int qr = n + (i >> 3);
-            *reinterpret_cast<u32x4_t*>(O + (base_row + qr) * a.ldo + h * HD + (i & 7) * 8) = u32x4_t{0u, 0u, 0u, 0u};
+            *reinterpret_cast<u32x4_t*>(O + (size_t)qr * a.ldo + (i & 7) * 8) = u32x4_t{0u, 0u, 0u, 0u};
         }
     }
 
@@ -257,7 +256,7 @@
         idx = ok ? idx : NK * 8 - 1;
         const int key = idx >> 3, c = idx & 7;
         const int kr = key < n ? key : n - 1;
-        const u32x4_t kc = *reinterpret_cast<const u32x4_t*>(K + (base_row + kr) * a.ldk + h * HD + c * 8);
+        const u32x4_t kc = *reinterpret_cast<const u32x4_t*>(K + (size_t)kr * a.ldk + c * 8);
         if (ok) *reinterpret_cast<u32x4_t*>(Ks + key * FA_LDK + c * 8) = kc;
     }
 #pragma unroll
@@ -271,7 +270,7 @@
         for (int e = 0; e < 4; ++e) {
             const int key = kg * 4 + e;
             const int kr = key < n ? key : n - 1;
-            vc[e] = *reinterpret_cast<const u32x4_t*>(V + (base_row + kr) * a.ldv + h * HD + c * 8);
+            vc[e] = *reinterpret_cast<const u32x4_t*>(V + (size_t)kr * a.ldv + c * 8);
             if (key >= n) vc[e] = u32x4_t{0u, 0u, 0u, 0u};
         }
         if (ok) {
@@ -299,7 +298,7 @@
         for (int u = 0; u < NT; ++u) {
             int qr = (t0 + 4 * u) * 16 + l15;
             qr = qr < n ? qr : n - 1;
-            const bf16_t* qp = Q + (base_row + qr) * a.ldq + h * HD + lg * 8;
+            const bf16_t* qp = Q + (size_t)qr * a.ldq + lg * 8;
             qf[u][0] = *reinterpret_cast<const bf16x8_t*>(qp);
             qf[u][1] = *reinterpret_cast<const bf16x8_t*>(qp + 32);
         }
@@ -392,7 +391,7 @@
         for (int u = 0; u < NT; ++u) {
             const int qr = (t0 + 4 * u) * 16 + l15;
             if (qr < n) {
-                bf16_t* op = O + (base_row + qr) * a.ldo + h * HD;
+                bf16_t* op = O + (size_t)qr * a.ldo;
 #pragma unroll
                 for (int dt = 0; dt < 4; ++dt) {
                     uint2 tt;
@@ -684,8 +683,17 @@
     }
 }
 
-hipError_t launch_attn_full(const AttnFullArgs& a, int B, bool is_f32, int impl, hipStream_t s) {
+bool attn_full_short_form(int N) { const int nsub = (N + 15) / 16; return nsub == 13 || nsub == 17; }
+
+hipError_t launch_attn_full(const AttnFullArgs& a_in, int B, bool is_f32, int impl, hipStream_t s) {
+    AttnFullArgs a = a_in;
     if (B <= 0 || a.N <= 0) return hipSuccess;
+    const bool blocked = a.hs_q || a.hs_k || a.hs_v || a.hs_o || a.is_q || a.is_k || a.is_v || a.is_o;
+    if (blocked && (impl != 1 || is_f32 || a.ntok || !attn_full_short_form(a.N))) return hipErrorInvalidValue;
+    if (!blocked) {
+        a.hs_q = a.hs_k = a.hs_v = a.hs_o = HD;
+        a.is_q = (long long)a.N * a.ldq; a.is_k = (long long)a.N * a.ldk; a.is_v = (long long)a.N * a.ldv; a.is_o = (long long)a.N * a.ldo;
+    }
     if (impl == 1) {
         if (is_f32) return hipErrorInvalidValue;
         const int nsub = (a.N + 15) / 16;
diff --git a/generativeimage2text_amd/csrc/kernels_gemm.hip b/generativeimage2text_amd/csrc/kernels_gemm.hip
--- a/generativeimage2text_amd/csrc/kernels_gemm.hip
+++ b/generativeimage2text_amd/csrc/kernels_gemm.hip
@@ -291,6 +291,7 @@
     if (g.out_f16 && (in_f32 || out_f32 || g.K % 64 != 0)) return hipErrorInvalidValue;
     if (gemm_uses_p8(g, in_f32, out_f32)) return launch_gemm_p8(g, out_f32, s);
     if (g.ln_part || g.part_out || g.res_part) return hipErrorInvalidValue;
+    if (g.blk_cols || g.a_blk) return hipErrorInvalidValue;
     if (g.out_f16) return launch_gemm_tiles<bf16_t, f16_t>(g, s);
     if (in_f32) {
         if (g.K % 16 != 0) return hipErrorInvalidValue;
diff --git a/generativeimage2text_amd/csrc/kernels_gemm10.hip b/generativeimage2text_amd/csrc/kernels_gemm10.hip
--- a/generativeimage2text_amd/csrc/kernels_gemm10.hip
+++ b/generativeimage2text_amd/csrc/kernels_gemm10.hip
@@ -122,6 +122,14 @@
 
     const char* __restrict__ Ab = reinterpret_cast<const char*>(g.A);
     const char* __restrict__ Wb = reinterpret_cast<const char*>(g.W);
+    uint32_t k_a_magic = g.a_magic, k_a_rs = g.a_rs, k_a_kt = g.a_kt, k_blk_tokens = (uint32_t)g.blk_tokens;
+    asm volatile("" : "+s"(Ab), "+s"(Wb), "+s"(k_a_magic), "+s"(k_a_rs), "+s"(k_a_kt), "+s"(k_blk_tokens));
+    uint32_t k_blk_cols = 0, k_blk_magic = 0;
+    void* k_Cb = nullptr;
+    if constexpr (sizeof(TOut) == 2 && LNF != 2) {
+        k_blk_cols = (uint32_t)g.blk_cols; k_blk_magic = g.blk_magic; k_Cb = g.Cb;
+        asm volatile("" : "+s"(k_blk_cols), "+s"(k_blk_magic), "+s"(k_Cb));
+    }
 
     const int Rl = lane >> 4, hi = (lane >> 3) & 1, lo = lane & 7;
     uint32_t a_off[2][2], w_off[2][2];
@@ -133,13 +141,15 @@
             const int ch = lo ^ (q * 4 + Rl);
             int m = m0 + rr;
             m = m < g.M ? m : g.M - 1;
-            a_off[h][q] = ((uint32_t)m * (uint32_t)g.lda + ch * 8) * 2u;
+            const uint32_t img = __umulhi((uint32_t)m, k_a_magic), tok = (uint32_t)m - img * k_blk_tokens;
+            a_off[h][q] = (img * (k_blk_tokens * (uint32_t)g.lda) + tok * k_a_rs + ch * 8) * 2u;
             const int rn = h * 128 + (wave * 2 + q) * 8 + 2 * Rl + (hi ^ q);
             w_off[h][q] = ((uint32_t)(n0 + rn) * (uint32_t)g.K + ch * 8) * 2u;
         }
+    const uint32_t a_kt = k_a_kt;
     auto issue = [&](int isw, int half, int kt) {
         if constexpr (DBG & 8) return;
-        const char* src = (isw ? Wb : Ab) + (size_t)kt * (BK * 2);
+        const char* src = isw ? Wb + (size_t)kt * (BK * 2) : Ab + (size_t)kt * a_kt;
         unsigned char* dst = smem + (kt & 1) * BUF_BYTES + (isw ? SLOT_B0 : SLOT_A0) + half * HALF_BYTES + wave * 2048;
         const uint32_t o0 = isw ? w_off[half][0] : a_off[half][0];
         const uint32_t o1 = isw ? w_off[half][1] : a_off[half][1];
@@ -401,6 +411,8 @@
                 }
             }
             P8_LDS_BARRIER();
+            auto copy_out = [&](auto blk_c) {
+            constexpr bool BLK = decltype(blk_c)::value;
 #pragma unroll 4
             for (int q = 0; q < MHq * CPR / 512; ++q) {
                 const int chunk = tid + q * 512;
@@ -439,6 +451,13 @@
                             for (int e = 0; e < 4; ++e) v[e] = pack2o<TOut>(f[2 * e], f[2 * e + 1]);
                         }
                         TOut* cp = C + (size_t)m * g.ldc + n;
+                        if constexpr (BLK) {
+                            uint32_t nb = (uint32_t)n;
+                            asm volatile("" : "+v"(nb));
+                            const uint32_t img = __umulhi((uint32_t)m, k_blk_magic), tok = (uint32_t)m - img * k_blk_tokens;
+                            cp = reinterpret_cast<TOut*>(k_Cb) +
+                                 ((size_t)(img * (k_blk_cols >> 6) + (nb >> 6)) * k_blk_tokens + tok) * 64 + (nb & 63);
+                        }
                         if (g.dbg & 512)
                             *reinterpret_cast<u32x4_t*>(cp) = v;
                         else
@@ -491,6 +510,13 @@
                         asm volatile("global_store_dwordx4 %0, %1, off sc1\n\ts_nop 1" ::"v"(cp), "v"(v) : "memory");
                     }
                 }
+            }
+            };
+            if constexpr (sizeof(TOut) == 2 && LNF != 2) {
+                if (n0 < (int)k_blk_cols) copy_out(std::true_type{});
+                else copy_out(std::false_type{});
+            } else {
+                copy_out(std::false_type{});
             }
             P8_LDS_BARRIER();
         }
@@ -592,6 +618,17 @@
     else launch_p8_t<float, MH, 1, MH1>(g, s);
 }
 
+bool gemm_p8_blocked_ok(const GemmArgs& g, bool out_f32) {
+    if (!g.blk_cols && !g.a_blk) return true;
+    if (g.blk_tokens < 2 || g.M % g.blk_tokens || (unsigned long long)g.M * (unsigned)g.blk_tokens >= 0x100000000ull) return false;
+    if (g.blk_cols) {
+        if (out_f32 || g.out_f16 || g.res || g.part_out || g.res_part || !g.Cb || (reinterpret_cast<uintptr_t>(g.Cb) & 15)) return false;
+        if (g.blk_cols < 0 || g.blk_cols % BN || g.blk_cols > g.N) return false;
+    }
+    if (g.a_blk && g.lda != g.K) return false;
+    return true;
+}
+
 hipError_t launch_gemm_p8(GemmArgs g, bool out_f32, hipStream_t s) {
     if (g.ln_part || g.part_out || g.res_part) {
 #ifndef GITMI_OPS_F16
@@ -601,6 +638,11 @@
         if ((g.part_out || g.res_part) && (!g.out_f16 || out_f32 || g.act != 0 || g.N > 1024)) return hipErrorInvalidValue;
         if (g.res_part && (!g.res || !g.res_gamma || !g.res_beta || g.res_nparts < 1)) return hipErrorInvalidValue;
     }
+    if (!gemm_p8_blocked_ok(g, out_f32)) return hipErrorInvalidValue;
+    g.blk_magic = g.blk_tokens ? (unsigned)(0x100000000ull / (unsigned)g.blk_tokens) + 1u : 0u;
+    g.a_magic = g.a_blk ? g.blk_magic : 0u;
+    g.a_rs = g.a_blk ? BK : (unsigned)g.lda;
+    g.a_kt = (g.a_blk ? (unsigned)g.blk_tokens : 1u) * (BK * 2);
     static const int heights[5] = {256, 224, 192, 160, 128};
     int bm = 256;
     if (!g.shared) {
diff --git a/generativeimage2text_amd/csrc/launchers.h b/generativeimage2text_amd/csrc/launchers.h
--- a/generativeimage2text_amd/csrc/launchers.h
+++ b/generativeimage2text_amd/csrc/launchers.h
@@ -17,11 +17,14 @@
     const float2* ln_part; int ln_nparts; const float* ln_colsum; float ln_inv_d, ln_eps;
     float2* part_out;
     const float2* res_part; int res_nparts; const float* res_gamma; const float* res_beta; float res_inv_d, res_eps;
+    int blk_tokens, blk_cols, a_blk; void* Cb;
+    unsigned blk_magic, a_magic, a_rs, a_kt;
 };
 bool gemm_uses_p8(const GemmArgs& g, bool in_f32, bool out_f32);
 hipError_t launch_gemm(const GemmArgs& g, bool in_f32, bool out_f32, hipStream_t s);
 hipError_t launch_gemm_p8(GemmArgs g, bool out_f32, hipStream_t s);
 bool gemm_p8_supports(const GemmArgs& g);
+bool gemm_p8_blocked_ok(const GemmArgs& g, bool out_f32);
 int gemm_p8_cost(const GemmArgs& g, int bm);
 bool set_gemm_impl(int impl);
 
@@ -158,8 +161,28 @@
     int N, H;
     float scale;
     const int* ntok;
+    int hs_q, hs_k, hs_v, hs_o;
+    long long is_q, is_k, is_v, is_o;
 };
 hipError_t launch_attn_full(const AttnFullArgs& a, int B, bool is_f32, int impl, hipStream_t s);
+inline AttnFullArgs attn_full_blocked_args(const void* q, const void* kv_rows, void* out, int width, int heads, int N) {
+    const long long head = (long long)N * 64, image = (long long)N * width;
+    AttnFullArgs a{};
+    a.q = q; a.out = out;
+    a.ldq = a.ldo = 64; a.hs_q = a.hs_o = (int)head; a.is_o = image;
+    if (kv_rows) {
+        a.k = (const unsigned short*)kv_rows + width;
+        a.v = (const unsigned short*)kv_rows + 2 * (size_t)width;
+        a.ldk = a.ldv = 3 * width; a.hs_k = a.hs_v = 64; a.is_k = a.is_v = 3 * image; a.is_q = image;
+    } else {
+        a.k = (const unsigned short*)q + image;
+        a.v = (const unsigned short*)q + 2 * image;
+        a.ldk = a.ldv = 64; a.hs_k = a.hs_v = (int)head; a.is_q = a.is_k = a.is_v = 3 * image;
+    }
+    a.N = N; a.H = heads; a.scale = 0.125f;
+    return a;
+}
+bool attn_full_short_form(int N);
 
 struct AttnDecodeArgs {
     const void* qkv; const void* img_k; const void* img_v; void* txt_k; void* txt_v; void* out;
diff --git a/generativeimage2text_amd/engine.py b/generativeimage2text_amd/engine.py
--- a/generativeimage2text_amd/engine.py
+++ b/generativeimage2text_amd/engine.py
@@ -1196,6 +1196,31 @@
     return out
 
 
+class blocked_ops:
+
+    def __init__(self, tokens: int, cols: int = 0, a: bool = False):
+        self.value = f"{int(tokens)},{int(cols)},{int(bool(a))}"
+
+    def __enter__(self):
+        os.environ["GITMI_OP_BLOCKED"] = self.value
+        return self
+
+    def __exit__(self, *exc):
+        os.environ.pop("GITMI_OP_BLOCKED", None)
+
+
+def op_attention_blocked(qkv: torch.Tensor, B: int, N: int, H: int, cols: int) -> torch.Tensor:
+    lib = _exp_library(qkv.dtype)
+    if lib not in (_libs.get("exp"), _libs.get("f16_exp")):
+        raise GitmiError("op_attention_blocked needs the measurement build: call use_experiment_build() first")
+    D = H * 64
+    assert qkv.is_cuda and qkv.is_contiguous() and qkv.numel() == B * N * (3 * D if cols == 3 * D else 4 * D)
+    out = torch.empty(B, H, N, 64, device=qkv.device, dtype=qkv.dtype)
+    with blocked_ops(N, cols):
+        _ck(lib.gitmi_op_attention(qkv.data_ptr(), out.data_ptr(), B, N, H, _torch_dtype_code(qkv), 1, _stream()), lib)
+    return out
+
+
 def strip_stats(x: torch.Tensor) -> torch.Tensor:
     M, N = x.shape
     xs = x.float().reshape(M, N // 16, 16)
```

After: 11580 captions/s. -1.8%, worse.
